# ZijiaLewisLu/CVPR2025-DeCafNet

Measured on AMD Instinct MI355X. Metric: clips/sec (grounding fwd, T=16384 D=1024), higher is better.
Workload: dtype f32; 1 GPU; BASELINE configs[2]: T=16384 D=1024 full multi-scale pyramid + sidekick top-k 30% + expert path, NQ=1 queries/video, 24 independent videos per step: 3 forwards in flight on 3 HIP streams x 8 videos per forward, one replica of this per GPU; T=16384, vid_len=16384, D=1024, E=256, TE=256, levels=8, win=9, heads=4, fusion_layers=2, sn=60, msf=True, norm=True, Lq=32, nq=1, max_batch=8, forwards_in_flight=3

## Files before the change

### cvpr2025-decafnet_amd/_lib.py

```python
import ctypes
import os

_HERE = os.path.dirname(os.path.abspath(__file__))
SO_PATH = os.environ.get('DCF_LIB_PATH') or os.path.join(_HERE, 'libdecafnet_hip.so')
_LIB = None

c_f32p = ctypes.c_void_p
c_u8p = ctypes.c_void_p
c_i32p = ctypes.c_void_p
c_i64p = ctypes.c_void_p
i32, i64, f32, f64 = ctypes.c_int32, ctypes.c_int64, ctypes.c_float, ctypes.c_double
vp = ctypes.c_void_p


class DcfConfig(ctypes.Structure):
    _fields_ = [(n, i32) for n in ('D', 'E', 'TE', 'vid_heads', 'fusion_heads', 'fusion_layers', 'n_embd_convs',
                                   'n_stem', 'n_levels', 'win', 'head_layers', 'sn')] + \
               [('sratio', f32)] + [(n, i32) for n in ('msf', 'norm', 'use_abs_pe', 'max_batch', 'gemm_mode', 'model_kind', 'second_fusion',
                                                      'text_in', 'text_layers', 'text_heads', 'text_abs_pe', 'text_bkgd',
                                                      'scat', 'sfonly', 'text_kind', 'xattn_affine', 'vid_stride', 'pool_only', 'attn_mode')]


class DcfOptimGroup(ctypes.Structure):
    _fields_ = [(n, f32) for n in ('lr', 'weight_decay', 'b1', 'b2', 'one_minus_b1', 'one_minus_b2', 'eps', 'bc1', 'sqrt_bc2')] + [('mode', i32)]
# ... 98 lines not shown
    'dcf_op_decoder': (i32, [vp, ctypes.c_char_p, c_f32p, c_u8p, i32, i32, ctypes.POINTER(vp), ctypes.POINTER(vp), ctypes.POINTER(i32), vp]),
    'dcf_op_tcn': (i32, [vp, ctypes.c_char_p, c_f32p, c_u8p, i32, i32, i32, i32, c_f32p, vp]),
    'dcf_optim_grad_norm': (i32, [vp, c_i32p, i32, i64, f32, c_f32p, c_f32p, vp]),
    'dcf_optim_scale': (i32, [vp, c_i32p, i32, i64, c_f32p, vp]),
    'dcf_optim_adam_step': (i32, [vp, c_i32p, i32, i64, vp, i32, c_f32p, i32, f32, vp]),
}

_DROP = [i32, i32, i32, i32, i64, i32, f32]
TRAIN_SIGNATURES = {
    'dcf_train_ext_version': (i32, []),
    'dcf_op_dropout': (i32, [c_f32p, c_f32p] + _DROP + [vp]),
    'dcf_op_gelu_dropout': (i32, [c_f32p, c_f32p] + _DROP + [vp]),
    'dcf_op_gelu_dropout_bwd': (i32, [c_f32p, c_f32p, c_f32p] + _DROP + [vp]),
    'dcf_op_drop_residual': (i32, [c_f32p, c_u8p, c_f32p, c_u8p, c_f32p, c_f32p] + _DROP + [i32, f32, vp]),
    'dcf_op_drop_residual_bwd': (i32, [c_f32p, c_f32p, c_u8p, c_u8p, c_f32p, c_f32p, c_f32p, c_f32p] + _DROP + [i32, f32, i32, vp]),
}


DIST_SIGNATURES = {
    'dcf_dist_ext_version': (i32, []),
    'dcf_dist_pack_grads': (i32, [vp, c_i32p, i32, i64, f32, vp]),
}


ATTN_SIGNATURES = {
    'dcf_attn_ext_version': (i32, []),
    'dcf_op_global_attn_bwd': (i32, [c_f32p, c_f32p, c_f32p, c_u8p, c_f32p, c_f32p, c_f32p, c_f32p, i32, i32, i32, i32, vp]),
}


FRONT_NO_SKIP = 1
FRONT_SIGNATURES = {
    'dcf_front_ext_version': (i32, []),
    'dcf_op_vidmap_shared': (i32, [c_f32p, c_f32p, c_f32p, c_f32p, c_f32p, c_u8p, c_f32p, c_i32p, c_f32p, i32, i32, i32, i32, i32, vp]),
    'dcf_op_vidmap_shared_bwd': (i32, [c_f32p, c_f32p, c_f32p, c_u8p, c_f32p, c_i32p, c_f32p, c_f32p, c_f32p, i32, i32, i32, i32, i32, i32, vp]),
}


GUARD_APPLY, GUARD_SKIP = 0, 1


class DcfGuardState(ctypes.Structure):
    _fields_ = [('verdict', i32), ('first_bad_row', i32), ('n_bad_rows', i32), ('reserved0', i32), ('applied', i64), ('skipped', i64),
                ('last_skipped_attempt', i64), ('conv_flag', i32), ('reserved1', i32)]


GUARD_SIGNATURES = {
    'dcf_guard_ext_version': (i32, []),
    'dcf_guard_grad_norm': (i32, [vp, c_i32p, i32, i64, f32, c_f32p, c_f32p, vp, vp]),
    'dcf_guard_adam_step': (i32, [vp, c_i32p, i32, i64, vp, i32, c_f32p, vp, i32, f32, vp]),
    'dcf_guard_arm': (i32, [vp, vp]),
    'dcf_guard_disarm': (i32, [vp]),
}


CLOCK_MAX_TABLE = 1 << 22
CLOCK_SIGNATURES = {
    'dcf_clock_ext_version': (i32, []),
    'dcf_clock_adam_step': (i32, [vp, c_i32p, i32, i64, vp, i32, vp, c_i32p, c_i64p, c_f32p, vp, i32, f32, vp]),
}


c_f16p = ctypes.c_void_p
HALF_SIGNATURES = {
    'dcf_half_ext_version': (i32, []),
    'dcf_forward_eval_h': (i32, [vp, c_f16p, c_f16p, c_u8p, i64, i32, ctypes.POINTER(vp), ctypes.POINTER(vp),
                                 ctypes.POINTER(i32), c_f32p, c_f32p, c_f32p, c_u8p, vp]),
    'dcf_forward_eval_videos_h': (i32, [vp, i32, ctypes.POINTER(vp), ctypes.POINTER(vp), ctypes.POINTER(vp), i64, ctypes.POINTER(i32),
                                        ctypes.POINTER(vp), ctypes.POINTER(vp), ctypes.POINTER(i32), ctypes.POINTER(vp),
                                        c_f32p, c_f32p, c_u8p, vp]),
    'dcf_op_linear_cm_split_h': (i32, [c_f16p, c_f32p, c_f32p, c_f32p, i32, i32, i32, i32, i32, vp]),
    'dcf_op_linear_cm_split_ld_h': (i32, [c_f16p, i64, c_f32p, c_f32p, c_f32p, i32, i32, i32, i32, i32, vp]),
    'dcf_op_sidekick_h': (i32, [c_f16p, c_f32p, c_f32p, i32, i32, i32, i32, vp]),
}


FRONT_HALF_SIGNATURES = {
    'dcf_front_half_ext_version': (i32, []),
    'dcf_op_vidmap_shared_h': (i32, [c_f16p, c_f16p, c_f32p, c_f32p, c_f32p, c_u8p, c_f32p, c_i32p, c_f32p, i32, i32, i32, i32, i32, vp]),
    'dcf_op_vidmap_shared_bwd_h': (i32, [c_f16p, c_f16p, c_f32p, c_u8p, c_f32p, c_i32p, c_f32p, c_f32p, c_f32p, i32, i32, i32, i32, i32, i32, vp]),
}


def lib():
    global _LIB
    if _LIB is None:
        import torch
        if not os.path.exists(SO_PATH):
            raise RuntimeError(f'{SO_PATH} is missing: build it with __graft_entry__.build() '
                               f'(there is no CPU fallback for the grounding path)')
        h = ctypes.CDLL(SO_PATH, mode=ctypes.RTLD_GLOBAL)
        for name, (res, args) in list(SIGNATURES.items()) + list(TRAIN_SIGNATURES.items()) + list(DIST_SIGNATURES.items()) + \
                list(ATTN_SIGNATURES.items()) + list(FRONT_SIGNATURES.items()) + list(GUARD_SIGNATURES.items()) + list(CLOCK_SIGNATURES.items()) + \
                list(HALF_SIGNATURES.items()) + list(FRONT_HALF_SIGNATURES.items()):
            fn = getattr(h, name)
            fn.restype = res
            fn.argtypes = args
        _LIB = h
    return _LIB


def check(rc, what=''):
    if rc != 0:
        msg = lib().dcf_last_error().decode(errors='replace')
        raise RuntimeError(f'decafnet_hip {what} failed: {msg}')


def ptr(t):
    return None if t is None else ctypes.c_void_p(t.data_ptr())


def current_stream():
    import torch
    return ctypes.c_void_p(torch.cuda.current_stream().cuda_stream)
```

### cvpr2025-decafnet_amd/csrc/engine.h

```cpp
#pragma once
#include <string>
#include <unordered_map>
#include <vector>

#include "../../include/decafnet_hip.h"
#include "attn.h"
#include "attn_grad.h"
#include "common.h"
#include "dec_chain.h"
#include "dropout.h"
#include "enc_chain.h"
#include "ffn_chain.h"
#include "gemm.h"
#include "head_chain.h"
#include "heads.h"
#include "postproc.h"
#include "rowops.h"
#include "score.h"

namespace dcf {

struct Bound {
  const float* p = nullptr;
  std::vector<int64_t> shape;
  int64_t numel() const {
    int64_t n = 1;
    for (auto s : shape) n *= s;
    return n;
  }
};

struct EncW {
  const float *ln_attn_w, *ln_attn_b, *dw_q, *dw_k, *dw_v, *qn_w, *qn_b, *kn_w, *kn_b, *vn_w, *vn_b;
  const float *wq, *bq, *wk, *bk, *wv, *bv, *wp, *bp, *ls_attn;
  const float *ln_ffn_w, *ln_ffn_b, *fc_w, *fc_b, *pj_w, *pj_b, *ls_ffn;
  const float *fc_wf, *fc_s, *fc_c;
  const unsigned short* qkv_chain[3];
  const float *qkv_s[3], *qkv_c[3];
  const unsigned short* wp_chain;
};
struct DecW {
  const float *ln_q_w, *ln_q_b, *ln_kv_w, *ln_kv_b, *dw, *qn_w, *qn_b;
  const float *wq, *bq, *wk, *bk, *wv, *bv, *wp, *bp;
  const float *wp_il, *bp_il;
  const float *ln_ffn_w, *ln_ffn_b, *fc_w, *fc_b, *pj_w, *pj_b, *ls_ffn;
  const float *fc_wf, *fc_s, *fc_c;
  const unsigned short *wq_chain, *wp_chain;
};
struct TextEncW {
  const float *ln_attn_w, *ln_attn_b, *wq, *bq, *wk, *bk, *wv, *bv, *wp, *bp, *ls_attn;
  const float *ln_ffn_w, *ln_ffn_b, *fc_w, *fc_b, *pj_w, *pj_b, *ls_ffn;
};
struct HeadW {
  std::vector<const float*> conv;
  std::vector<const float*> ln_w, ln_b;
  const float* out_w;
  const float* out_b;
  const unsigned short* chain[2] = {nullptr, nullptr};
  const unsigned short* out_chain = nullptr;
};

static inline int vid_stride_of(const dcf_config& c) { return c.vid_stride > 1 ? c.vid_stride : 1; }

struct Plan {
  int T0 = 0, B = 0, L = 0;
  LevelTable lt{};
  LevelTable* d_lt = nullptr;
};

struct HybridState;

}

struct dcf_model {
  dcf_config cfg{};
  std::unordered_map<std::string, dcf::Bound> bound;
  std::vector<float*> owned;
  std::unordered_map<const float*, const unsigned short*> wsplit;
  std::unordered_map<const float*, int64_t> wsplit_ldw;
  std::unordered_map<const float*, int> wsplit_terms;
  int gemm_terms = 16;
  bool force_x6 = false;
  bool no_ln_carry = false;
  int option_epoch = 0;
  unsigned* status = nullptr;
  bool finalized = false;
  const float* pe = nullptr;
  int64_t pe_T = 0;

  const float *vid_map_w = nullptr, *vid_map_b = nullptr;
  const float *vid_w1 = nullptr, *vid_w2 = nullptr, *vid_w3 = nullptr;
  int64_t vid_ldw = 0;
  std::vector<dcf::DecW> dec;
  const float *fus_out_w = nullptr, *fus_out_b = nullptr;
  const float *embd_fc_w = nullptr, *embd_fc_b = nullptr;
  const float *embd_fc_wf = nullptr, *embd_fc_s = nullptr, *embd_fc_c = nullptr;
  std::vector<const float*> embd_conv, embd_ln_w, embd_ln_b;
  std::vector<dcf::EncW> stem, branch;
  std::vector<const float*> pool_w;
  dcf::HeadW cls1, cls2, reg;
  std::vector<float> reg_scales;
  const float *tcn_in_w = nullptr, *tcn_in_b = nullptr, *tcn_out_w = nullptr, *tcn_out_b = nullptr;
  std::vector<const float*> tcn_wd, tcn_bd, tcn_wp, tcn_bp, tcn_lnw, tcn_lnb;
  std::vector<const unsigned short*> tcn_frag;
  const float *text_embd_w = nullptr, *text_embd_b = nullptr, *text_bkgd = nullptr;
  dcf::TextEncW text_pool{};
  std::vector<dcf::TextEncW> text_enc;
  const float* text_pe = nullptr;
  int64_t text_pe_L = 0;
  char* text_ws = nullptr;
  size_t text_ws_bytes = 0;
  char* half_ws = nullptr;
  size_t half_ws_bytes = 0;

  char* arena = nullptr;
  size_t arena_bytes = 0;
  std::vector<dcf::Plan> plans;
  std::vector<uint64_t> last_key, graph_key;
  hipGraph_t graph = nullptr;
  hipGraphExec_t graph_exec = nullptr;
  bool capturing = false;
  int graph_mode = 0;
  std::vector<uint64_t> nocapture_key;
  int last_launch = 0;
  hipStream_t own = nullptr;
  hipEvent_t ev_in = nullptr, ev_out = nullptr;
  struct {
    float *correl = nullptr, *gate = nullptr, *vidmap = nullptr, *fused = nullptr, *F = nullptr;
    int nq = 0, T0 = 0, B = 0, S = 0;
  } dbg;
  dcf::HybridState* hyb = nullptr;
  int hyb_levels = 0;
  size_t hyb_extra = 0;
  char* hyb_extra_ptr = nullptr;
  float* hyb_feat_out = nullptr;
  float* dbg_vidmap = nullptr;
  float* dbg_fused = nullptr;
  int64_t dbg_cap = 0;
  bool keep_debug = false;
  struct DropState {
    float p[5] = {0.f, 0.f, 0.f, 0.f, 0.f};
    float scale[5] = {1.f, 1.f, 1.f, 1.f, 1.f};
    uint64_t seed = 0;
    bool active = false;
    int b0 = 0;
  } drop_state;
  DropState* drop = nullptr;
};

namespace dcf {

struct Arena {
  char* base;
  size_t off = 0, cap;
  bool dry;
  template <typename T>
  T* take(size_t n) {
    off = (off + 255) & ~(size_t)255;
    T* p = dry ? nullptr : reinterpret_cast<T*>(base + off);
    off += n * sizeof(T);
    return p;
  }
};

struct Buffers {
  float *P1, *P2, *tn, *partial, *correl, *gate;
  uint8_t *mask_all, *nbr_all, *kvmask, *maskv;
  uint8_t* tile_flags;
  uint8_t *mask_pre, *nbr_pre;
  float* col5;
  float *X, *R[7], *H2, *HID, *F, *HA, *HB, *HC, *HD, *logits1, *tcnA, *tcnB, *kvn, *Kt, *Vt;
  unsigned short* kvimg;
  float* kmadd;
  float* stats;
  float* hstats[2];
};

constexpr int DCF_MAX_VIDEOS = 16;
struct VideoSet {
  int nvid = 0;
  const float* vid[DCF_MAX_VIDEOS];
  const float* shallow[DCF_MAX_VIDEOS];
  const uint8_t* mask[DCF_MAX_VIDEOS];
  const float* text_cls[DCF_MAX_VIDEOS];
  int nq[DCF_MAX_VIDEOS];
  float* logits1_out = nullptr;
  bool half = false;
};

struct ForwardCall {
  const float* const* text; const uint8_t* const* text_mask; const int32_t* text_len;
  const float* gate;
  float *logits, *offsets; uint8_t* masks;
};

struct HybridState {
  bool valid = false;
  int k = 0, Tn = 0, Tc = 0, B = 0, Lk = 0;
  Buffers bn{};
  Plan pn{}, pc{}, pch{};
  float *Fc = nullptr, *logits1c = nullptr, *stacked = nullptr;
  uint8_t *maskc = nullptr, *nbrc = nullptr;
};

static inline GemmArgs gemm(const float* A, int64_t lda, const float* W, const float* bias, float* C, int64_t ldc, int M, int N,
                            int K) {
  GemmArgs g{};
  g.A = A; g.lda = lda; g.W = W; g.ldw = 0; g.bias = bias; g.C = C; g.ldc = ldc; g.M = M; g.N = N; g.K = K;
  return g;
}

#define TRY(x) do { if ((x) != 0) return -1; } while (0)
constexpr int STATS_W = 64;
enum { DROP_R_VPROJ = 0, DROP_R_VPATH, DROP_R_FPROJ, DROP_R_FPATH, DROP_R_REFINE };

const char* last_error();
int debug_option(const char* name, int dflt);
int option_epoch();
bool profiling_on();
class Setting {
 public:
  enum Kind { VALUE, PRESENT };
  Setting(const char* opt, const char* env, int dflt, Kind kind = VALUE);
  int get() const;
 private:
  const char* opt_; int base_;
};
void launch_permute3(const float* src, float* dst, int d0, int d1, int d2, int p0, int p1, int p2, hipStream_t st);
void launch_fold_ln(const float* W, const float* bias, const float* g, const float* beta, float* Wf, float* s, float* c, int N, int K,
                    hipStream_t st);
void drop_graph(dcf_model* m, bool keep_last_key = false);
void free_packed(dcf_model* m);
int init_gemm_mode(dcf_model* m, hipStream_t st);
int resolve_encoder(dcf_model* m, const std::string& p, int E, hipStream_t st, EncW& w);
int resolve_decoder(dcf_model* m, const std::string& p, int E, int TE, hipStream_t st, DecW& w);
int resolve_tcn(dcf_model* m, const std::string& pre, int n_in, int n_layers, hipStream_t st);

size_t carve_at(char* base, const dcf_config& c, int T0, int B, int nq, int S, int Lk, int nvid, Buffers& b, size_t extra = 0,
                char** extra_ptr = nullptr);
int get_plan(dcf_model* m, int T0, int B, int L, hipStream_t st, Plan** out);
int make_plan(dcf_model* m, Plan& p, const int* Tl, int n, int B, const float* scales, hipStream_t st);
int run_gemm(dcf_model* m, GemmArgs* g, int count, GemmAMode mode, hipStream_t st);
bool can_fuse_ln(dcf_model* m, const float* W, int M, int N, int K, GemmAMode mode);
bool can_norm_a(dcf_model* m, const float* W1, const float* W2, int M, int C, int* stats_w);
void norm_a(GemmArgs& g, const float* stats, int C, int stats_w, const float* ln_g, const float* ln_b);
EncPreArgs enc_pre_args(const EncW& w, const float* X, int64_t ldx, const uint8_t* mask_in, int B, int T_in, int E);
int run_encoder(dcf_model* m, const EncW& w, Buffers& b, const float* Xin, int64_t ldx, const uint8_t* mask_in,
                const uint8_t* mask_out, int B, int T_in, int stride, float* Xout, int64_t ldo, hipStream_t st);
int run_encoder_drop(dcf_model* m, const EncW& w, Buffers& b, const float* Xin, int64_t ldx, const uint8_t* mask_in,
                     const uint8_t* mask_out, int B, int T_in, int stride, float* Xout, int64_t ldo, uint32_t site0, hipStream_t st);
int run_head(dcf_model* m, const HeadW& h, Buffers& b, const Plan& pl, int Cin, int NO, int mode, int query_major, float* out,
             hipStream_t st, int row0 = 0, int rows = -1);
int run_head_pair(dcf_model* m, const HeadW& h1, const HeadW& h2, Buffers& b, const Plan& pl, int Cin, int NO1, int mode1,
                  float* out1, int NO2, int mode2, float* out2, hipStream_t st);
int run_fusion(dcf_model* m, Buffers& b, float* X, int64_t ldx, int B, int T, const LevelTable* lt, const uint8_t* mask,
               const uint8_t* nbr, const TextMeta* dm, int Lk, float* out, int64_t ld_out, hipStream_t st, bool* carry_out = nullptr);
int run_fusion_drop(dcf_model* m, Buffers& b, float* X, int64_t ldx, int B, int T, const uint8_t* mask, const TextMeta* dm, int Lk,
                    float* out, int64_t ld_out, hipStream_t st);
RefineArgs refine_args(dcf_model* m);

int forward(dcf_model* m, const VideoSet& vs, int T0, int nq, const ForwardCall& fc, hipStream_t st);
void launch_masks_out(const uint8_t* mask_all, uint8_t* out, const LevelTable* lt, const unsigned* status, float* logits, int rows,
                      hipStream_t st);

int launch_half_to_f32(const uint16_t* src, float* dst, int64_t n, hipStream_t st);

void free_hybrid(dcf_model* m);
int hybrid_take(dcf_model* m, const Buffers& b, const Plan& pl, int B, int Lk, hipStream_t st);

}
```

### cvpr2025-decafnet_amd/csrc/engine.hip

```cpp
#include <algorithm>

#include "engine.h"
#include "../../include/decafnet_hip_half.h"

namespace dcf {

__global__ void k_masks_out(const uint8_t* __restrict__ mask_all, uint8_t* __restrict__ out, const LevelTable* lt,
                            const unsigned* __restrict__ status, float* __restrict__ logits) {
  const int r = blockIdx.x * blockDim.x + threadIdx.x;
  const int total = lt->start[lt->n_levels];
  if (r >= total) return;
  int l = 0;
  while (l + 1 < lt->n_levels && r >= lt->start[l + 1]) ++l;
  const int rel = r - lt->start[l];
  const int b = rel / lt->T[l], t = rel - b * lt->T[l];
  const int64_t o = (int64_t)b * lt->S + lt->off[l] + t;
  out[o] = mask_all[r];
  if (status && (status[0] & 3u)) logits[o] = __uint_as_float(0x7fc00000u);
}
void launch_masks_out(const uint8_t* mask_all, uint8_t* out, const LevelTable* lt, const unsigned* status, float* logits, int rows,
                      hipStream_t st) {
  hipLaunchKernelGGL(k_masks_out, dim3((rows + 255) / 256), dim3(256), 0, st, mask_all, out, lt, status, logits);
}

// ... 181 lines not shown
    if (gate_first) {
      if (m->vid_w2) for (int v = 0; v < nvid; ++v) TRY(shallow_half(v));
      TRY(flush());
      TRY(gather_masks());
      GateArgs ga{b.correl, nvid > 1 ? b.maskv : vid_mask, b.gate, sv > 1 ? b.mask_pre : b.mask_all, T0, nq, 0, c.sn, c.msf, (double)c.sratio, vmap0,
                  b.tile_flags, nflags};
      TRY(launch_gate(ga, st));
      auto wit = m->wsplit.find(m->vid_w1);
      const bool one_grid = nvid > 1 && nvid <= GEMM_ZMAX && E % 256 == 0 && T0 % 4 == 0 && wit != m->wsplit.end() && m->wsplit_ldw[m->vid_w1] == m->vid_ldw;
      if (one_grid) {
        GemmArgs base = gemm(vs.vid[0], T0, m->vid_w1, nullptr, b.P1, E, T0, E, D);
        base.ldw = m->vid_ldw; base.a_scale = 1.f; base.Ws = wit->second; base.status = m->status; base.skip_stride = nflags;
        const float* zA[GEMM_ZMAX]; float* zC[GEMM_ZMAX]; const uint8_t* zs[GEMM_ZMAX]; int zq[GEMM_ZMAX];
        for (int v = 0; v < nvid; ++v) { zA[v] = vs.vid[v]; zC[v] = b.P1 + (size_t)v * T0 * E; zs[v] = b.tile_flags + (size_t)q_of[v] * nflags; zq[v] = vs.nq[v]; }
        TRY(launch_gemm_split_z(base, nvid, zA, zC, zs, zq, m->wsplit_terms[m->vid_w1], st, std::min(1.0, std::max(0.0, (double)c.sratio)),
                                half_native ? A_CHANMAJOR_H : A_CHANMAJOR));
      } else {
        for (int v = 0; v < nvid; ++v) TRY(expert_half(v, true));
        TRY(flush());
      }
    } else {
      for (int v = 0; v < nvid; ++v) {
        if (m->vid_w1) TRY(expert_half(v, false));
        if (m->vid_w2) TRY(shallow_half(v));
      }
      TRY(flush());
      TRY(gather_masks());
    }
  }
  if (nvid > 1) vid_mask = b.maskv;

  for (int q0 = 0; q0 < nq; q0 += Bmax) {
    const int B = std::min(Bmax, nq - q0);
    Plan* pl;
    TRY(get_plan(m, Tp, B, L, st, &pl));
    const LevelTable& lt = pl->lt;
    const int rows0 = B * T0, rowsP = B * Tp, rowsAll = B * S;
    uint8_t* mask_in = sv > 1 ? b.mask_pre : b.mask_all;
    if (m->drop) m->drop->b0 = q0;
    unsigned long long vmap = 0;
    for (int i = 0; i < B && i < 16; ++i) vmap |= (unsigned long long)video_of[q0 + i] << (4 * i);

    if (fc.gate) {
      hipLaunchKernelGGL(k_apply_gate, dim3((rows0 + 255) / 256), dim3(256), 0, st, fc.gate + (int64_t)q0 * T0, vid_mask,
                         b.gate, mask_in, T0, rows0, c.msf);
      DCF_HIP(hipGetLastError());
    } else if (!gate_first) {
      GateArgs ga{b.correl, vid_mask, b.gate, mask_in, T0, B, q0, c.sn, c.msf, (double)c.sratio, vmap, nullptr, 0};
      TRY(launch_gate(ga, st));
    }
    int pre_off = 0;
    if (sv > 1) {
      int rows_pre = 0;
      for (int j = 0; j <= npre; ++j) { if (j == npre) pre_off = rows_pre; rows_pre += B * (T0 >> j); }
      TRY(launch_pyramid_masks(b.mask_pre, b.nbr_pre, B, T0, npre + 1, rows_pre, st));
      DCF_HIP(hipMemcpyAsync(b.mask_all, b.mask_pre + pre_off, (size_t)rowsP, hipMemcpyDeviceToDevice, st));
    }
    TRY(launch_pyramid_masks(b.mask_all, b.nbr_all, B, Tp, L, rowsAll, st));
    const uint8_t* mask0 = mask_in;
    const uint8_t* maskP = b.mask_all;

    TRY(launch_vidmap_combine(m->vid_w1 ? b.P1 : nullptr, m->vid_w2 ? b.P2 : nullptr, m->vid_map_b, b.gate, mask0,
                              m->vid_w3, m->vid_w3 ? b.correl + (int64_t)q0 * T0 : nullptr, b.X, T0, rows0, E, vmap, st));
    if (m->keep_debug) DCF_CHECK((int64_t)rows0 * E <= m->dbg_cap, "dcf_debug_copy: armed destination holds %lld floats, the tap needs %lld", (long long)m->dbg_cap, (long long)rows0 * E);
    if (m->keep_debug && m->dbg_vidmap) DCF_HIP(hipMemcpyAsync(m->dbg_vidmap, b.X, (size_t)rows0 * E * 4, hipMemcpyDeviceToDevice, st));

    TextMeta tm{};
    for (int i = 0; i < B; ++i) {
      tm.text[i] = fc.text[q0 + i];
      tm.text_mask[i] = fc.text_mask ? fc.text_mask[q0 + i] : nullptr;
      tm.len[i] = fc.text_len[q0 + i];
    }
    const TextMeta* dm = &tm;

    bool fused_as_stats = false;
    if (c.model_kind != 1) {
      const bool tap = m->keep_debug && m->dbg_fused;
      if (m->drop) TRY(run_fusion_drop(m, b, b.X, E, B, T0, mask0, dm, Lk, b.R[0], E, st));
      else TRY(run_fusion(m, b, b.X, E, B, T0, nullptr, mask0, nullptr, dm, Lk, b.R[0], E, st, tap ? nullptr : &fused_as_stats));
      if (tap) DCF_HIP(hipMemcpyAsync(m->dbg_fused, b.R[0], (size_t)rows0 * E * 4, hipMemcpyDeviceToDevice, st));
    }

    {
      if (c.model_kind != 1 && fused_as_stats) {
        GemmArgs ge = gemm(b.X, E, m->embd_fc_wf, m->embd_fc_c, b.R[3], E, rows0, E, E);
        ge.flags = G_AMASK; ge.rowmask = mask0;
        ge.stats_in = b.stats; ge.ln_s = m->embd_fc_s; ge.stats_slots = E / STATS_W; ge.stats_w = STATS_W;
        TRY(run_gemm(m, &ge, 1, A_ROWS, st));
        std::swap(b.X, b.R[3]);
      } else if (c.model_kind != 1) {
        GemmArgs ge = gemm(b.R[0], E, m->embd_fc_w, m->embd_fc_b, b.X, E, rows0, E, E);
        ge.flags = G_AMASK; ge.rowmask = mask0;
        TRY(run_gemm(m, &ge, 1, A_ROWS, st));
      }
      if (sv > 1) {
        int Tc = T0, off = 0;
        for (int i = 0; i < c.n_embd_convs; ++i) {
          const bool with_pe = c.use_abs_pe && i == c.n_embd_convs - 1;
          if (Tc > Tp) {
            TRY(launch_im2col5s2(b.X, E, b.mask_pre + off, b.col5, B, Tc, E, st));
            GemmArgs g = gemm(b.col5, 5 * E, m->embd_conv[i], nullptr, b.R[0], E, B * (Tc / 2), E, 5 * E);
            TRY(run_gemm(m, &g, 1, A_ROWS, st));
            off += B * Tc;
            Tc /= 2;
          } else {
            GemmArgs g = gemm(b.X, E, m->embd_conv[i], nullptr, b.R[0], E, B * Tc, E, 3 * E);
            g.cin = E; g.nbr = b.nbr_pre + off;
            TRY(run_gemm(m, &g, 1, A_ROWS_TAP3, st));
          }
          LnArgs ln{}; ln.X = b.R[0]; ln.ldx = E; ln.Y = b.X; ln.ldy = E; ln.w = m->embd_ln_w[i]; ln.b = m->embd_ln_b[i];
          ln.rows = B * Tc; ln.C = E; ln.relu = 1;
          if (with_pe) { ln.pe = m->pe; ln.mask = b.mask_pre + off; ln.T = Tc; }
          TRY(launch_ln(ln, st));
        }
        DCF_CHECK(Tc == Tp, "vid_net.arch[0]=%d embedding convolutions cannot divide the sequence by vid_net.stride=%d (video_net.py:53)", c.n_embd_convs, sv);
      }
      int epend = -1, epend_w = 0;
      for (int i = 0; i < c.n_embd_convs && sv == 1; ++i) {
        GemmArgs g = gemm(b.X, E, m->embd_conv[i], nullptr, b.R[0], E, rows0, E, 3 * E);
        g.cin = E; g.nbr = b.nbr_all;
        const bool with_pe = c.use_abs_pe && i == c.n_embd_convs - 1;
        int sw = 0;
        if (epend >= 0) {
          g.A = b.R[0]; g.C = b.R[3];
          norm_a(g, b.hstats[0], E, epend_w, m->embd_ln_w[epend], m->embd_ln_b[epend]);
          epend = -1;
          TRY(run_gemm(m, &g, 1, A_ROWS_TAP3, st));
          LnArgs ln{}; ln.X = b.R[3]; ln.ldx = E; ln.Y = b.X; ln.ldy = E; ln.w = m->embd_ln_w[i]; ln.b = m->embd_ln_b[i];
          ln.rows = rows0; ln.C = E; ln.relu = 1;
          if (with_pe) { ln.pe = m->pe; ln.mask = mask0; ln.T = T0; }
          TRY(launch_ln(ln, st));
        } else if (i + 1 < c.n_embd_convs && i + 2 == c.n_embd_convs && can_norm_a(m, m->embd_conv[i], m->embd_conv[i + 1], rows0, E, &sw)) {
          g.stats_out = b.hstats[0]; g.stats_w = sw;
          TRY(run_gemm(m, &g, 1, A_ROWS_TAP3, st));
          epend = i; epend_w = sw;
        } else
        if (can_fuse_ln(m, m->embd_conv[i], rows0, E, 3 * E, A_ROWS_TAP3)) {
          g.C = nullptr; g.ln_w = m->embd_ln_w[i]; g.ln_b = m->embd_ln_b[i]; g.Y = b.R[3]; g.ldy = E; g.ln_relu = 1;
          if (with_pe) { g.ln_pe = m->pe; g.ln_mask = mask0; g.ln_T = T0; }
          TRY(run_gemm(m, &g, 1, A_ROWS_TAP3, st));
          std::swap(b.X, b.R[3]);
        } else {
          TRY(run_gemm(m, &g, 1, A_ROWS_TAP3, st));
          LnArgs ln{}; ln.X = b.R[0]; ln.ldx = E; ln.Y = b.X; ln.ldy = E; ln.w = m->embd_ln_w[i]; ln.b = m->embd_ln_b[i];
          ln.rows = rows0; ln.C = E; ln.relu = 1;
          if (with_pe) { ln.pe = m->pe; ln.mask = mask0; ln.T = T0; }
          TRY(launch_ln(ln, st));
        }
      }
      if (c.use_abs_pe && c.n_embd_convs == 0) {
        LnArgs ln{}; ln.X = b.X; ln.ldx = E; ln.Y = b.X; ln.ldy = E; ln.rows = rows0; ln.C = E; ln.skip_ln = 1;
        ln.pe = m->pe; ln.mask = mask0; ln.T = T0;
        TRY(launch_ln(ln, st));
      }
      for (size_t i = 0; i < m->stem.size(); ++i) {
        if (m->drop) TRY(run_encoder_drop(m, m->stem[i], b, b.X, E, maskP, maskP, B, Tp, 1, b.R[3], E, drop_site(DROP_G_STEM, (uint32_t)i, 0), st));
        else TRY(run_encoder(m, m->stem[i], b, b.X, E, maskP, maskP, B, Tp, 1, b.R[3], E, st));
        DCF_HIP(hipMemcpyAsync(b.X, b.R[3], (size_t)rowsP * E * 4, hipMemcpyDeviceToDevice, st));
      }
      const int ldf = E + TCN_HID;
      const float* xin = b.X;
      int64_t ldx = E;
      for (int l = 0; l < L; ++l) {
        const int stride = l > 0 ? 2 : 1;
        const uint8_t* mi = b.mask_all + lt.start[l > 0 ? l - 1 : 0];
        const uint8_t* mo = b.mask_all + lt.start[l];
        float* xo = b.F + (int64_t)lt.start[l] * ldf;
        if (c.pool_only) TRY(launch_dwconv3(xin, ldx, mi, m->pool_w[l], xo, ldf, B, l > 0 ? lt.T[l - 1] : Tp, stride, E, st));
        else if (m->drop) TRY(run_encoder_drop(m, m->branch[l], b, xin, ldx, mi, mo, B, l > 0 ? lt.T[l - 1] : Tp, stride, xo, ldf,
                                               drop_site(DROP_G_BRANCH, (uint32_t)l, 0), st));
        else TRY(run_encoder(m, m->branch[l], b, xin, ldx, mi, mo, B, l > 0 ? lt.T[l - 1] : Tp, stride, xo, ldf, st));
        xin = xo; ldx = ldf;
      }
    }

    if (m->hyb_levels > 0) {
      TRY(hybrid_take(m, b, *pl, B, Lk, st));
      continue;
    }

    if (c.model_kind == 1 || c.second_fusion)
      TRY(run_fusion(m, b, b.F, E + TCN_HID, B, Tp, &lt, b.mask_all, b.nbr_all, dm, Lk, b.F, E + TCN_HID, st));

    if (c.model_kind != 0) {
      TRY(run_head_pair(m, m->cls1, m->reg, b, *pl, E, 1, 0, fc.logits + (int64_t)q0 * S, 2, 1, fc.offsets + (int64_t)q0 * S * 2, st));
    } else {
    TRY(run_head(m, m->cls1, b, *pl, E, 1, 0, 0, b.logits1, st));
    if (vs.logits1_out) {
      hipLaunchKernelGGL(k_points_out, dim3((rowsAll + 255) / 256), dim3(256), 0, st, (const float*)b.logits1,
                         vs.logits1_out + (int64_t)q0 * S, (const LevelTable*)pl->d_lt);
      DCF_HIP(hipGetLastError());
    }
    {
      RefineArgs ra = refine_args(m);
      ra.logits1 = b.logits1; ra.lt = pl->d_lt; ra.mask_all = b.mask_all;
      ra.bufA = b.tcnA; ra.bufB = b.tcnB; ra.F = b.F; ra.ldf = E + TCN_HID; ra.E = E;
      ra.B = B; ra.T0 = Tp; ra.n_levels = L; ra.n_layers = L;
      if (m->drop) {
        ra.drop_seed = m->drop->seed; ra.drop_p = m->drop->p[DROP_R_REFINE]; ra.drop_scale = m->drop->scale[DROP_R_REFINE]; ra.drop_b0 = q0;
      }
      TRY(launch_refine(ra, lt, st));
// ... 291 lines not shown
```

### cvpr2025-decafnet_amd/csrc/engine_blocks.hip

```cpp
#include <algorithm>

#include "engine.h"

namespace dcf {

static void carve(Arena& a, const dcf_config& c, int T0, int B, int nq, int S, int Lk, int nvid, Buffers& b) {
  const size_t rows0 = (size_t)B * T0, rowsAll = (size_t)B * S;
  const size_t rowsF = std::max(rows0, (c.model_kind == 1 || c.second_fusion) ? rowsAll : (size_t)0);
  const bool strided = vid_stride_of(c) > 1;
  const int E = c.E, EH = c.E + TCN_HID;
  b.P1 = a.take<float>((size_t)nvid * T0 * E);
  b.P2 = a.take<float>((size_t)nvid * T0 * E);
  b.maskv = a.take<uint8_t>(nvid > 1 ? (size_t)nvid * T0 : 0);
  b.tn = a.take<float>((size_t)nq * c.D);
  b.partial = a.take<float>((size_t)SCORE_SLICES * (nq + nvid) * T0);
  b.correl = a.take<float>((size_t)nq * T0);
  b.gate = a.take<float>(rows0);
  b.tile_flags = a.take<uint8_t>((size_t)B * ((T0 + 63) / 64));
  b.mask_all = a.take<uint8_t>(rowsAll);
  b.nbr_all = a.take<uint8_t>(rowsAll);
  b.mask_pre = a.take<uint8_t>(strided ? 2 * rows0 : 0);
  b.nbr_pre = a.take<uint8_t>(strided ? 2 * rows0 : 0);
  b.col5 = a.take<float>(strided ? rows0 / 2 * 5 * E : 0);
  b.kvmask = a.take<uint8_t>((size_t)B * Lk);
// ... 463 lines not shown
  }
  if (!m->fus_out_w) return 0;
  LnArgs ln{}; ln.X = X; ln.ldx = ldx; ln.Y = out; ln.ldy = ld_out; ln.w = m->fus_out_w; ln.b = m->fus_out_b; ln.rows = rows; ln.C = E;
  TRY(launch_ln(ln, st));
  return 0;
}

static DropSite drop_at(const dcf_model* m, int rate, uint32_t site) {
  DropSite d;
  d.site = site; d.p = m->drop->p[rate]; d.scale = m->drop->scale[rate];
  return d;
}

int run_encoder_drop(dcf_model* m, const EncW& w, Buffers& b, const float* Xin, int64_t ldx, const uint8_t* mask_in,
                     const uint8_t* mask_out, int B, int T_in, int stride, float* Xout, int64_t ldo, uint32_t site0,
                     hipStream_t st) {
  const dcf_config& c = m->cfg;
  const int E = c.E, To = T_in / stride, rows = B * To;
  const auto& d = *m->drop;
  TRY(enc_unfused_qkv(m, w, b, Xin, ldx, mask_in, B, T_in, stride, st));
  TRY(enc_unfused_attention(m, b, mask_out, B, To, st));
  GemmArgs gp = gemm(b.R[0], E, w.wp, w.bp, b.R[4], E, rows, E, E);
  TRY(run_gemm(m, &gp, 1, A_ROWS, st));
  DropResArgs ra{};
  ra.out = b.R[1]; ra.ldo = E;
  if (stride == 2) { ra.R = b.R[3]; ra.ldr = E; } else { ra.R = Xin; ra.ldr = ldx; }
  ra.H = b.R[4]; ra.ldh = E; ra.rowmask = mask_out; ra.res_mask = 1; ra.out_mask = 0; ra.ls = w.ls_attn;
  ra.rows = rows; ra.C = E; ra.T = To; ra.b0 = d.b0; ra.seed = d.seed;
  ra.drop = drop_at(m, DROP_R_VPROJ, site0 | DROP_PROJ); ra.path = drop_at(m, DROP_R_VPATH, site0 | DROP_PATH_ATTN);
  TRY(launch_drop_residual(ra, st));
  LnArgs ln{}; ln.X = b.R[1]; ln.ldx = E; ln.Y = b.R[2]; ln.ldy = E; ln.w = w.ln_ffn_w; ln.b = w.ln_ffn_b; ln.rows = rows; ln.C = E;
  TRY(launch_ln(ln, st));
  GemmArgs gf = gemm(b.R[2], E, w.fc_w, w.fc_b, b.HID, 4 * E, rows, 4 * E, E);
  gf.flags = G_GELU;
  TRY(run_gemm(m, &gf, 1, A_ROWS, st));
  TRY(launch_dropout(b.HID, 4 * E, rows, 4 * E, To, d.b0, d.seed, drop_at(m, DROP_R_VPROJ, site0 | DROP_FFN_HID), st));
  GemmArgs go = gemm(b.HID, 4 * E, w.pj_w, w.pj_b, b.R[4], E, rows, E, 4 * E);
  TRY(run_gemm(m, &go, 1, A_ROWS, st));
  ra.out = Xout; ra.ldo = ldo; ra.R = b.R[1]; ra.ldr = E; ra.res_mask = 0; ra.out_mask = 1; ra.ls = w.ls_ffn;
  ra.drop = drop_at(m, DROP_R_VPROJ, site0 | DROP_FFN_OUT); ra.path = drop_at(m, DROP_R_VPATH, site0 | DROP_PATH_FFN);
  return launch_drop_residual(ra, st);
}

int run_fusion_drop(dcf_model* m, Buffers& b, float* X, int64_t ldx, int B, int T, const uint8_t* mask, const TextMeta* dm,
                    int Lk, float* out, int64_t ld_out, hipStream_t st) {
  const dcf_config& c = m->cfg;
  const int E = c.E, rows = B * T;
  const auto& d = *m->drop;
  for (size_t li = 0; li < m->dec.size(); ++li) {
    const DecW& w = m->dec[li];
    const uint32_t site0 = drop_site(DROP_G_FUSION, (uint32_t)li, 0);
    TextLnArgs tl{*dm, b.kvn, b.kvmask, w.ln_kv_w, w.ln_kv_b, Lk, c.TE};
    TRY(launch_text_ln(tl, B, st));
    GemmArgs gkv[2] = {gemm(b.kvn, c.TE, w.wk, w.bk, b.Kt, E, B * Lk, E, c.TE), gemm(b.kvn, c.TE, w.wv, w.bv, b.Vt, E, B * Lk, E, c.TE)};
    TRY(run_gemm(m, gkv, 2, A_ROWS, st));
    DecPreArgs dp{X, ldx, mask, w.ln_q_w, w.ln_q_b, w.dw, w.qn_w, w.qn_b, b.R[0], b.R[1], B, T, E};
    dp.nbr = nullptr;
    dp.affine = c.xattn_affine;
    TRY(launch_dec_pre(dp, st));
    GemmArgs gq = gemm(b.R[0], E, w.wq, w.bq, b.R[2], E, rows, E, E);
    TRY(run_gemm(m, &gq, 1, A_ROWS, st));
    XAttnArgs xa{b.R[2], b.Kt, b.Vt, b.kvmask, b.R[0], B, T, Lk, E, c.fusion_heads, m->status, c.attn_mode == 1};
    TRY(launch_xattn(xa, st));
    GemmArgs gh = gemm(b.R[0], E, w.wp, w.bp, b.H2, 2 * E, rows, 2 * E, E);
    TRY(run_gemm(m, &gh, 1, A_ROWS, st));
    TRY(launch_dropout(b.H2, 2 * E, rows, 2 * E, T, d.b0, d.seed, drop_at(m, DROP_R_FPROJ, site0 | DROP_PROJ), st));
    TRY(launch_dec_mid(b.R[1], b.H2, w.ln_ffn_w, w.ln_ffn_b, b.R[2], b.R[0], rows, E, st));
    GemmArgs gf = gemm(b.R[0], E, w.fc_w, w.fc_b, b.HID, 4 * E, rows, 4 * E, E);
    gf.flags = G_GELU;
    TRY(run_gemm(m, &gf, 1, A_ROWS, st));
    TRY(launch_dropout(b.HID, 4 * E, rows, 4 * E, T, d.b0, d.seed, drop_at(m, DROP_R_FPROJ, site0 | DROP_FFN_HID), st));
    GemmArgs go = gemm(b.HID, 4 * E, w.pj_w, w.pj_b, b.R[1], E, rows, E, 4 * E);
    TRY(run_gemm(m, &go, 1, A_ROWS, st));
    DropResArgs ra{};
    ra.out = X; ra.ldo = ldx; ra.R = b.R[2]; ra.ldr = E; ra.H = b.R[1]; ra.ldh = E; ra.rowmask = mask; ra.res_mask = 0; ra.out_mask = 1;
    ra.ls = w.ls_ffn; ra.rows = rows; ra.C = E; ra.T = T; ra.b0 = d.b0; ra.seed = d.seed;
    ra.drop = drop_at(m, DROP_R_FPROJ, site0 | DROP_FFN_OUT); ra.path = drop_at(m, DROP_R_FPATH, site0 | DROP_PATH_FFN);
    TRY(launch_drop_residual(ra, st));
  }
  LnArgs ln{}; ln.X = X; ln.ldx = ldx; ln.Y = out; ln.ldy = ld_out; ln.w = m->fus_out_w; ln.b = m->fus_out_b; ln.rows = rows; ln.C = E;
  return launch_ln(ln, st);
}

RefineArgs refine_args(dcf_model* m) {
  static const Setting stack("tcn_stack", "DCF_TCN_STACK", -1);
  RefineArgs ra{};
  ra.w_in = m->tcn_in_w; ra.b_in = m->tcn_in_b;
  ra.host_w_dil = m->tcn_wd.data(); ra.host_b_dil = m->tcn_bd.data(); ra.host_w_pw = m->tcn_wp.data();
  ra.host_b_pw = m->tcn_bp.data(); ra.host_ln_w = m->tcn_lnw.data(); ra.host_ln_b = m->tcn_lnb.data();
  ra.w_out = m->tcn_out_w; ra.b_out = m->tcn_out_b;
  ra.host_frag = (!m->tcn_frag.empty() && debug_option("tcn_frag", 1) != 0) ? m->tcn_frag.data() : nullptr;
  ra.stack_layers = stack.get();
  ra.f16 = m->gemm_terms == GEMM_F16X3; ra.status = m->status;
  return ra;
}

}
```

### cvpr2025-decafnet_amd/csrc/engine_model.hip

```cpp
#include <cstdarg>
#include <cstdio>
#include <cstdlib>
#include <algorithm>
#include <cstring>
#include <atomic>
#include <mutex>

#include "engine.h"

namespace dcf {

static thread_local std::string g_err;
void set_error(const char* fmt, ...) {
  char buf[1024];
  va_list ap;
  va_start(ap, fmt);
  vsnprintf(buf, sizeof(buf), fmt, ap);
  va_end(ap);
  g_err = buf;
}
const char* last_error() { return g_err.c_str(); }

static std::unordered_map<std::string, int>& debug_options() {
  static std::unordered_map<std::string, int> o;
  return o;
}
static std::mutex& debug_options_mutex() {
  static std::mutex mu;
  return mu;
}
static std::atomic<int> g_option_epoch{0};
int option_epoch() { return g_option_epoch.load(); }
int debug_option(const char* name, int dflt) {
  std::lock_guard<std::mutex> lock(debug_options_mutex());
  auto& o = debug_options();
  auto it = o.find(name);
  return it == o.end() ? dflt : it->second;
}
Setting::Setting(const char* opt, const char* env, int dflt, Kind kind) : opt_(opt), base_(dflt) {
  const char* v = env ? getenv(env) : nullptr;
  if (v) base_ = kind == PRESENT ? 1 : atoi(v);
}
int Setting::get() const { return opt_ ? debug_option(opt_, base_) : base_; }

struct ProfRec { std::string name; hipEvent_t a, b; double flops, bytes; };
static bool g_prof_on = false;
static std::vector<ProfRec> g_recs;
bool profiling_on() { return g_prof_on; }

ProfScope::ProfScope(const char* name, hipStream_t s, double flops, double bytes) : idx(-1), st(s) {
  if (!g_prof_on) return;
  ProfRec r{name, nullptr, nullptr, flops, bytes};
  if (hipEventCreate(&r.a) != hipSuccess || hipEventCreate(&r.b) != hipSuccess) return;
  (void)hipEventRecord(r.a, st);
  g_recs.push_back(r);
  idx = (int)g_recs.size() - 1;
}
ProfScope::~ProfScope() {
  if (idx >= 0) (void)hipEventRecord(g_recs[idx].b, st);
}

__global__ void k_permute3(const float* __restrict__ src, float* __restrict__ dst, int d0, int d1, int d2, int p0, int p1,
                           int p2) {
  const int n = d0 * d1 * d2;
  const int i = blockIdx.x * blockDim.x + threadIdx.x;
  if (i >= n) return;
  int idx[3];
  idx[0] = i / (d1 * d2);
  idx[1] = (i / d2) % d1;
  idx[2] = i % d2;
  const int dims[3] = {d0, d1, d2};
  const int perm[3] = {p0, p1, p2};
  const int o = (idx[perm[0]] * dims[perm[1]] + idx[perm[1]]) * dims[perm[2]] + idx[perm[2]];
  dst[o] = src[i];
}
void launch_permute3(const float* src, float* dst, int d0, int d1, int d2, int p0, int p1, int p2, hipStream_t st) {
  const size_t n = (size_t)d0 * d1 * d2;
  hipLaunchKernelGGL(k_permute3, dim3((unsigned)((n + 255) / 256)), dim3(256), 0, st, src, dst, d0, d1, d2, p0, p1, p2);
}

__global__ __launch_bounds__(64) void k_fold_ln(const float* __restrict__ W, const float* __restrict__ bias, const float* __restrict__ g,
                                                const float* __restrict__ beta, float* __restrict__ Wf, float* __restrict__ s,
                                                float* __restrict__ c, int K) {
  const int n = blockIdx.x, lane = threadIdx.x;
  float a1 = 0.f, a2 = 0.f;
  for (int k = lane; k < K; k += 64) {
    const float w = W[(int64_t)n * K + k];
    const float wf = w * g[k];
    Wf[(int64_t)n * K + k] = wf;
    a1 += wf;
    a2 += beta[k] * w;
  }
  a1 = wave_sum(a1);
  a2 = wave_sum(a2);
  if (lane == 0) { s[n] = a1; c[n] = (bias ? bias[n] : 0.f) + a2; }
}
void launch_fold_ln(const float* W, const float* bias, const float* g, const float* beta, float* Wf, float* s, float* c, int N, int K,
                    hipStream_t st) {
  hipLaunchKernelGGL(k_fold_ln, dim3(N), dim3(64), 0, st, W, bias, g, beta, Wf, s, c, K);
}

void drop_graph(dcf_model* m, bool keep_last_key) {
  if (m->graph_exec) (void)hipGraphExecDestroy(m->graph_exec);
  if (m->graph) (void)hipGraphDestroy(m->graph);
  m->graph_exec = nullptr;
  m->graph = nullptr;
  m->graph_key.clear();
  if (!keep_last_key) m->last_key.clear();
}

void free_packed(dcf_model* m) {
  for (float* p : m->owned) (void)hipFree(p);
  m->owned.clear();
  m->wsplit.clear();
  m->wsplit_ldw.clear();
  m->wsplit_terms.clear();
}

static int free_model(dcf_model* m) {
  drop_graph(m);
  if (m->status) (void)hipFree(m->status);
  m->status = nullptr;
  free_packed(m);
  for (auto& pl : m->plans) if (pl.d_lt) (void)hipFree(pl.d_lt);
  m->plans.clear();
  free_hybrid(m);
  if (m->arena) (void)hipFree(m->arena);
  if (m->text_ws) (void)hipFree(m->text_ws);
  if (m->half_ws) (void)hipFree(m->half_ws);
  if (m->ev_in) (void)hipEventDestroy(m->ev_in);
  if (m->ev_out) (void)hipEventDestroy(m->ev_out);
  if (m->own) (void)hipStreamDestroy(m->own);
  return 0;
}

static int get(dcf_model* m, const std::string& name, std::initializer_list<int64_t> shape, const float** out) {
  auto it = m->bound.find(name);
  DCF_CHECK(it != m->bound.end(), "parameter '%s' is not bound", name.c_str());
  const Bound& b = it->second;
  int64_t want = 1;
  for (auto s : shape) want *= s;
  DCF_CHECK(b.numel() == want, "parameter '%s' has %lld elements, expected %lld", name.c_str(), (long long)b.numel(),
            (long long)want);
  *out = b.p;
  return 0;
}

static int pack3(dcf_model* m, const float* src, int d0, int d1, int d2, int p0, int p1, int p2, hipStream_t st,
                 const float** out) {
  float* dst = nullptr;
  const size_t n = (size_t)d0 * d1 * d2;
  DCF_HIP(hipMalloc(&dst, n * sizeof(float)));
  m->owned.push_back(dst);
  launch_permute3(src, dst, d0, d1, d2, p0, p1, p2, st);
  DCF_HIP(hipGetLastError());
  *out = dst;
  return 0;
}

static int split_weight(dcf_model* m, const float* W, int N, int K, hipStream_t st, int64_t ldw = 0, int terms = 0) {
  if (m->gemm_terms == 0 || m->wsplit.count(W)) return 0;
  if (!terms) terms = m->gemm_terms;
  unsigned short* planes = nullptr;
  DCF_HIP(hipMalloc(&planes, (size_t)3 * N * K * sizeof(unsigned short)));
  m->owned.push_back(reinterpret_cast<float*>(planes));
  if (launch_split_planes(W, planes, N, K, ldw ? ldw : K, st, terms, m->status ? m->status + 1 : nullptr)) return -1;
  m->wsplit[W] = planes;
  m->wsplit_ldw[W] = ldw ? ldw : K;
  m->wsplit_terms[W] = terms;
  return 0;
}
#define SPLIT(W, N, K) do { if (split_weight(m, (W), (N), (K), st)) return -1; } while (0)

static int fold_ln(dcf_model* m, const float* W, const float* bias, const float* g, const float* beta, int N, int K, hipStream_t st,
                   const float** wf, const float** s_out, const float** c_out) {
  float* buf = nullptr;
  DCF_HIP(hipMalloc(&buf, ((size_t)N * K + 2 * (size_t)N) * sizeof(float)));
  m->owned.push_back(buf);
  float* sv = buf + (size_t)N * K;
  launch_fold_ln(W, bias, g, beta, buf, sv, sv + N, N, K, st);
  DCF_HIP(hipGetLastError());
  *wf = buf; *s_out = sv; *c_out = sv + N;
// ... 208 lines not shown
      const std::string p = "text_net.attn_pool.attn";
      GET(p + ".query.weight", SH(TE, TE), w.wq); GET(p + ".query.bias", SH(TE), w.bq);
      GET(p + ".key.weight", SH(TE, TE), w.wk); GET(p + ".key.bias", SH(TE), w.bk);
      GET(p + ".value.weight", SH(TE, TE), w.wv); GET(p + ".value.bias", SH(TE), w.bv);
      GET(p + ".proj.weight", SH(TE, TE), w.wp); GET(p + ".proj.bias", SH(TE), w.bp);
      SPLIT(w.wq, TE, TE); SPLIT(w.wk, TE, TE); SPLIT(w.wv, TE, TE); SPLIT(w.wp, TE, TE);
    }
  } else
  if (c.text_layers > 0 || c.text_in > 0) {
    DCF_CHECK(c.text_in > 0 && c.text_layers >= 0 && c.text_heads >= 1 && TE % c.text_heads == 0,
              "text_net: in_dim=%d layers=%d heads=%d do not fit TE=%d", c.text_in, c.text_layers, c.text_heads, TE);
    GET("text_net.embd_fc.conv.weight", SH(TE, c.text_in), m->text_embd_w); GET("text_net.embd_fc.conv.bias", SH(TE), m->text_embd_b);
    if (c.text_bkgd) GET("text_net.bkgd_token", SH(TE), m->text_bkgd);
    for (int i = 0; i < c.text_layers; ++i) {
      const std::string p = "text_net.transformer." + std::to_string(i);
      TextEncW w{};
      GET(p + ".ln_attn.weight", SH(TE), w.ln_attn_w); GET(p + ".ln_attn.bias", SH(TE), w.ln_attn_b);
      GET(p + ".attn.attn.query.weight", SH(TE, TE), w.wq); GET(p + ".attn.attn.query.bias", SH(TE), w.bq);
      GET(p + ".attn.attn.key.weight", SH(TE, TE), w.wk); GET(p + ".attn.attn.key.bias", SH(TE), w.bk);
      GET(p + ".attn.attn.value.weight", SH(TE, TE), w.wv); GET(p + ".attn.attn.value.bias", SH(TE), w.bv);
      GET(p + ".attn.attn.proj.weight", SH(TE, TE), w.wp); GET(p + ".attn.attn.proj.bias", SH(TE), w.bp);
      GET(p + ".drop_path_attn.scale", SH(TE), w.ls_attn);
      GET(p + ".ln_ffn.weight", SH(TE), w.ln_ffn_w); GET(p + ".ln_ffn.bias", SH(TE), w.ln_ffn_b);
      GET(p + ".ffn.fc.weight", SH(4 * TE, TE), w.fc_w); GET(p + ".ffn.fc.bias", SH(4 * TE), w.fc_b);
      GET(p + ".ffn.proj.weight", SH(TE, 4 * TE), w.pj_w); GET(p + ".ffn.proj.bias", SH(TE), w.pj_b);
      GET(p + ".drop_path_ffn.scale", SH(TE), w.ls_ffn);
      SPLIT(w.wq, TE, TE); SPLIT(w.wk, TE, TE); SPLIT(w.wv, TE, TE); SPLIT(w.wp, TE, TE);
      SPLIT(w.fc_w, 4 * TE, TE); SPLIT(w.pj_w, TE, 4 * TE);
      m->text_enc.push_back(w);
    }
  }

  if (c.model_kind == 1) {
    GET("vid_net.embd_fc.conv.weight", SH(E, Din), m->vid_map_w); GET("vid_net.embd_fc.conv.bias", SH(E), m->vid_map_b);
  } else {
    GET("vid_map.conv.weight", SH(E, Din), m->vid_map_w); GET("vid_map.conv.bias", SH(E), m->vid_map_b);
  }
  m->vid_w1 = (c.msf && sfonly) ? nullptr : m->vid_map_w;
  m->vid_w2 = c.msf ? (sfonly ? m->vid_map_w : m->vid_map_w + D) : nullptr;
  m->vid_w3 = nullptr;
  m->vid_ldw = Din;
  if (c.scat) {
    float* blk[3] = {nullptr, nullptr, nullptr};
    const float* src[3] = {m->vid_w1, m->vid_w2, m->vid_map_w + (Din - 1)};
    const int wid[3] = {D, D, 1};
    for (int i = 0; i < 3; ++i) {
      if (!src[i]) continue;
      DCF_HIP(hipMalloc(&blk[i], (size_t)E * wid[i] * sizeof(float)));
      m->owned.push_back(blk[i]);
      DCF_HIP(hipMemcpy2DAsync(blk[i], (size_t)wid[i] * 4, src[i], (size_t)Din * 4, (size_t)wid[i] * 4, E, hipMemcpyDeviceToDevice, st));
    }
    m->vid_w1 = blk[0]; m->vid_w2 = blk[1]; m->vid_w3 = blk[2];
    m->vid_ldw = D;
  }
  if (D % 32 == 0 && E % 32 == 0) {
    if (m->vid_w1 && split_weight(m, m->vid_w1, E, D, st, m->vid_ldw)) return -1;
    if (m->vid_w2 && split_weight(m, m->vid_w2, E, D, st, m->vid_ldw)) return -1;
  }
  for (int i = 0; i < c.fusion_layers; ++i) {
    DecW w{};
    if (resolve_decoder(m, "fusion.layers." + std::to_string(i), E, TE, st, w)) return -1;
    m->dec.push_back(w);
  }
  GET("fusion.ln_out.weight", SH(E), m->fus_out_w); GET("fusion.ln_out.bias", SH(E), m->fus_out_b);
  if (c.model_kind != 1) {
    GET("vid_net.embd_fc.conv.weight", SH(E, E), m->embd_fc_w); GET("vid_net.embd_fc.conv.bias", SH(E), m->embd_fc_b);
    SPLIT(m->embd_fc_w, E, E);
    m->embd_fc_wf = m->embd_fc_s = m->embd_fc_c = nullptr;
    if (m->gemm_terms != 0 && E % 64 == 0 && c.fusion_layers > 0 &&
        fold_ln(m, m->embd_fc_w, m->embd_fc_b, m->fus_out_w, m->fus_out_b, E, E, st, &m->embd_fc_wf, &m->embd_fc_s, &m->embd_fc_c)) return -1;
  }
  for (int i = 0, sv = vid_stride_of(c); i < c.n_embd_convs; ++i, sv = std::max(sv / 2, 1)) {
    const std::string s = std::to_string(i);
    const int taps = sv > 1 ? 5 : 3;
    GET("vid_net.embd_convs." + s + ".conv.weight", SH(E, E, taps), t);
    const float* pk;
    if (pack3(m, t, E, E, taps, 0, 2, 1, st, &pk)) return -1;
    SPLIT(pk, E, taps * E);
    m->embd_conv.push_back(pk);
    const float *lw, *lb;
    GET("vid_net.embd_norms." + s + ".weight", SH(E), lw); GET("vid_net.embd_norms." + s + ".bias", SH(E), lb);
    m->embd_ln_w.push_back(lw); m->embd_ln_b.push_back(lb);
  }
  for (int i = 0; i < c.n_stem; ++i) {
    EncW w{};
    if (resolve_encoder(m, "vid_net.stem." + std::to_string(i), E, st, w)) return -1;
    m->stem.push_back(w);
  }
  m->pool_w.clear();
  for (int i = 0; i < L; ++i) {
    if (c.pool_only) {
      const float* pk;
      GET("vid_net.branch." + std::to_string(i) + ".conv.weight", SH(E, 3), t);
      if (pack3(m, t, 1, E, 3, 0, 2, 1, st, &pk)) return -1;
      m->pool_w.push_back(pk);
      continue;
    }
    EncW w{};
    if (resolve_encoder(m, "vid_net.branch." + std::to_string(i), E, st, w)) return -1;
    m->branch.push_back(w);
  }
  if (resolve_head(m, "cls_head", "cls_head", E, 1, c.head_layers, st, m->cls1)) return -1;
  const int EH = c.model_kind == 0 ? E + TCN_HID : E;
  if (c.model_kind == 0 && resolve_head(m, "cls_head2", "cls_head", EH, 1, c.head_layers, st, m->cls2)) return -1;
  if (resolve_head(m, "reg_head", "reg_head", EH, 2, c.head_layers, st, m->reg)) return -1;
  m->reg_scales.assign(L, 1.f);
  for (int l = 0; l < L; ++l) {
    GET("reg_head.scales." + std::to_string(l) + ".scale", SH(1), t);
    DCF_HIP(hipMemcpyAsync(&m->reg_scales[l], t, sizeof(float), hipMemcpyDeviceToHost, st));
  }
  if (c.model_kind == 0 && resolve_tcn(m, "refine", L, L, st)) return -1;
  DCF_HIP(hipStreamSynchronize(st));
  for (auto& pl : m->plans) if (pl.d_lt) (void)hipFree(pl.d_lt);
  m->plans.clear();
  free_hybrid(m);
  drop_graph(m);
  if (m->gemm_terms == GEMM_F16X3) {
    unsigned flags[2] = {0u, 0u};
    DCF_HIP(hipMemcpyAsync(flags, m->status, sizeof(flags), hipMemcpyDeviceToHost, st));
    DCF_HIP(hipStreamSynchronize(st));
    if (flags[1]) {
      m->force_x6 = true;
      return finalize(m, st);
    }
  }
  m->finalized = true;
  return 0;
}

}

extern "C" {

int dcf_model_create(const dcf_config* cfg, dcf_model** out) {
  DCF_CHECK(cfg && out, "dcf_model_create: null argument");
  DCF_CHECK(cfg->E > 0 && cfg->E % 32 == 0 && cfg->E <= 992, "E=%d must be a positive multiple of 32 (<= 992)", cfg->E);
  DCF_CHECK(cfg->attn_mode == 0 || cfg->attn_mode == 1, "attn_mode=%d: 0 (f16x3) or 1 (one fp16 product)", cfg->attn_mode);
  DCF_CHECK(cfg->D > 0 && cfg->D % 32 == 0, "D=%d must be a positive multiple of 32", cfg->D);
  DCF_CHECK(cfg->TE > 0 && cfg->TE % 32 == 0, "TE=%d must be a positive multiple of 32", cfg->TE);
  DCF_CHECK(cfg->n_levels >= 1 && cfg->n_levels <= dcf::DCF_MAX_LEVELS, "n_levels=%d out of range", cfg->n_levels);
  DCF_CHECK(cfg->win == 0 || (cfg->win > 0 && (cfg->win & 1)), "mha_win_size=%d must be odd, or 0 for global self-attention over the clips", cfg->win);
  DCF_CHECK(cfg->fusion_layers >= 0 && cfg->head_layers >= 0 && cfg->n_embd_convs >= 0 && cfg->n_stem >= 0, "negative layer count");
  DCF_CHECK(cfg->sn >= 1, "sn must be >= 1");
  DCF_CHECK(cfg->model_kind >= 0 && cfg->model_kind <= 2, "model_kind must be 0 (iterative early fusion), 1 (late fusion) or 2 (early fusion)");
  {
    const int sv = cfg->vid_stride > 1 ? cfg->vid_stride : 1;
    int lg = 0;
    while ((1 << lg) < sv) ++lg;
    DCF_CHECK((sv & (sv - 1)) == 0 && cfg->n_embd_convs >= lg, "vid_net.stride=%d must be a power of two with arch[0]=%d >= log2(stride) (video_net.py:52-53)",
              sv, cfg->n_embd_convs);
  }
  int ndev = 0;
  DCF_HIP(hipGetDeviceCount(&ndev));
  DCF_CHECK(ndev > 0, "no HIP device");
  dcf_model* m = new dcf_model();
  m->cfg = *cfg;
  *out = m;
  return 0;
}

void dcf_model_destroy(dcf_model* m) {
  if (!m) return;
  dcf::free_model(m);
  delete m;
}

int dcf_model_bind(dcf_model* m, const char* name, const float* data, const int64_t* shape, int32_t ndim) {
  DCF_CHECK(m && name && data, "dcf_model_bind: null argument");
  dcf::Bound b;
  b.p = data;
  for (int i = 0; i < ndim; ++i) b.shape.push_back(shape[i]);
  m->bound[name] = b;
  m->finalized = false;
  return 0;
}

int dcf_model_set_pe(dcf_model* m, const float* pe_tokens, int64_t T) {
  DCF_CHECK(m, "dcf_model_set_pe: null model");
  m->pe = pe_tokens;
  m->pe_T = T;
  return 0;
}

int dcf_model_set_text_pe(dcf_model* m, const float* pe_tokens, int64_t L) {
  DCF_CHECK(m, "dcf_model_set_text_pe: null model");
  m->text_pe = pe_tokens;
  m->text_pe_L = L;
  return 0;
}

int dcf_model_finalize(dcf_model* m, void* stream) {
  DCF_CHECK(m, "dcf_model_finalize: null model");
  return dcf::finalize(m, (hipStream_t)stream);
}

int dcf_numerics_status(dcf_model* m, int32_t reset, void* stream) {
  DCF_CHECK(m, "dcf_numerics_status: null model");
  int out = m->gemm_terms == dcf::GEMM_BF16X6 ? 4 : (m->gemm_terms == 0 ? 8 : 0);
  if (m->force_x6) out |= 2;
  if (m->status) {
    unsigned flag = 0u;
    hipStream_t st = (hipStream_t)stream;
    DCF_HIP(hipMemcpyAsync(&flag, m->status, sizeof(flag), hipMemcpyDeviceToHost, st));
    if (reset) DCF_HIP(hipMemsetAsync(m->status, 0, sizeof(unsigned), st));
    DCF_HIP(hipStreamSynchronize(st));
    if (flag & ~2u) out |= 1;
    if (flag & 2u) out |= 16;
  }
  return out;
}

int dcf_model_set_ln_carry(dcf_model* m, int32_t on) {
  DCF_CHECK(m, "dcf_model_set_ln_carry: null model");
  const bool off = on == 0;
  if (off != m->no_ln_carry) dcf::drop_graph(m);
  m->no_ln_carry = off;
  return 0;
}

int dcf_numerics_status_async(dcf_model* m, int32_t* host_dst, void* stream) {
  DCF_CHECK(m && host_dst, "dcf_numerics_status_async: null argument");
  if (!m->status) { *host_dst = 0; return 0; }
  DCF_HIP(hipMemcpyAsync(host_dst, m->status, sizeof(unsigned), hipMemcpyDeviceToHost, (hipStream_t)stream));
  return 0;
}

int dcf_model_set_dropout(dcf_model* m, float vid_proj_p, float vid_path_p, float fus_proj_p, float fus_path_p, float refine_p,
                          int64_t seed) {
  DCF_CHECK(m, "dcf_model_set_dropout: null model");
  const float p[5] = {vid_proj_p, vid_path_p, fus_proj_p, fus_path_p, refine_p};
  for (int i = 0; i < 5; ++i) DCF_CHECK(p[i] >= 0.f && p[i] < 1.f, "dcf_model_set_dropout: rate %d = %g outside [0, 1)", i, (double)p[i]);
  auto& d = m->drop_state;
  d.active = false;
  for (int i = 0; i < 5; ++i) {
    d.p[i] = p[i];
    d.scale[i] = 1.0f / (1.0f - p[i]);
    d.active = d.active || p[i] > 0.f;
  }
  d.seed = (uint64_t)seed;
  return 0;
}

int dcf_debug_set_option(const char* name, int32_t value) {
  DCF_CHECK(name && *name, "dcf_debug_set_option: empty name");
  static const char* known[] = {"dec_chain_min_rows", "enc_chain_min_rows", "enc_attn_min_rows", "fuse_scores", "tcn_frag", "gate_skip", "tcn_stack", "half_native"};
  bool ok = false;
  for (const char* k : known) ok = ok || strcmp(k, name) == 0;
  DCF_CHECK(ok, "dcf_debug_set_option: unknown option '%s'", name);
  {
    std::lock_guard<std::mutex> lock(dcf::debug_options_mutex());
    if (value < 0) dcf::debug_options().erase(name);
    else dcf::debug_options()[name] = value;
  }
  dcf::g_option_epoch.fetch_add(1);
  return 0;
}

int dcf_model_set_graph_mode(dcf_model* m, int32_t mode) {
  DCF_CHECK(m && mode >= 0 && mode <= 2, "dcf_model_set_graph_mode: mode must be 0 (auto), 1 (always) or 2 (never)");
  if (mode != m->graph_mode) dcf::drop_graph(m);
  m->graph_mode = mode;
  return 0;
}

int dcf_debug_copy(dcf_model* m, int32_t what, float* dst, int64_t max_floats, void* stream) {
  DCF_CHECK(m && dst, "dcf_debug_copy: null argument");
  hipStream_t st = (hipStream_t)stream;
  const float* src = nullptr;
  int64_t n = 0;
  const int E = m->cfg.E;
  switch (what) {
    case 0: src = m->dbg.correl; n = (int64_t)m->dbg.nq * m->dbg.T0; break;
    case 1: src = m->dbg.gate; n = (int64_t)m->dbg.B * m->dbg.T0; break;
    case 4: src = m->dbg.F; n = (int64_t)m->dbg.B * m->dbg.S * (E + dcf::TCN_HID); break;
    case 2: case 3: {
      m->keep_debug = true;
      m->dbg_cap = max_floats;
      if (what == 2) m->dbg_vidmap = dst; else m->dbg_fused = dst;
      return 0;
    }
    default: DCF_CHECK(false, "dcf_debug_copy: unknown selector %d", what);
  }
  DCF_CHECK(src, "dcf_debug_copy: no forward has run yet");
  DCF_CHECK(n <= max_floats, "dcf_debug_copy: destination too small (%lld > %lld)", (long long)n, (long long)max_floats);
  DCF_HIP(hipMemcpyAsync(dst, src, n * sizeof(float), hipMemcpyDeviceToDevice, st));
  return 0;
}

int dcf_profile_enable(int32_t on) {
  for (auto& r : dcf::g_recs) { (void)hipEventDestroy(r.a); (void)hipEventDestroy(r.b); }
  dcf::g_recs.clear();
  dcf::g_prof_on = on != 0;
  return 0;
}

int64_t dcf_profile_report(char* buf, int64_t cap) {
  struct Agg { long count = 0; double ms = 0, flops = 0, bytes = 0; };
  std::vector<std::pair<std::string, Agg>> aggs;
  for (auto& r : dcf::g_recs) {
    if (hipEventSynchronize(r.b) != hipSuccess) continue;
    float ms = 0.f;
    if (hipEventElapsedTime(&ms, r.a, r.b) != hipSuccess) continue;
    Agg* a = nullptr;
    for (auto& kv : aggs) if (kv.first == r.name) a = &kv.second;
    if (!a) { aggs.emplace_back(r.name, Agg()); a = &aggs.back().second; }
    a->count++; a->ms += ms; a->flops += r.flops; a->bytes += r.bytes;
  }
  std::string out = "{";
  for (size_t i = 0; i < aggs.size(); ++i) {
    char line[512];
    snprintf(line, sizeof(line), "%s\"%s\": {\"count\": %ld, \"ms\": %.6f, \"flops\": %.6e, \"bytes\": %.6e}", i ? ", " : "",
             aggs[i].first.c_str(), aggs[i].second.count, aggs[i].second.ms, aggs[i].second.flops, aggs[i].second.bytes);
    out += line;
  }
  out += "}";
  if (buf && cap > 0) {
    size_t n = std::min((size_t)cap - 1, out.size());
    memcpy(buf, out.data(), n);
    buf[n] = 0;
  }
  return (int64_t)out.size() + 1;
}

}
```

### cvpr2025-decafnet_amd/csrc/gemm_bf16s.hip

```cpp
#include <cstdio>
#include <type_traits>
#include <cstdlib>

#include "gemm_common.h"


namespace dcf {

typedef __bf16 bf16x8 __attribute__((ext_vector_type(8)));
typedef __bf16 bf16x2 __attribute__((ext_vector_type(2)));
typedef float f32x2 __attribute__((ext_vector_type(2)));
typedef unsigned int u32x4 __attribute__((ext_vector_type(4)));

typedef _Float16 f16x8 __attribute__((ext_vector_type(8)));
typedef _Float16 f16x2 __attribute__((ext_vector_type(2)));
typedef _Float16 f16x4 __attribute__((ext_vector_type(4)));

constexpr int SBK = 32;
constexpr int ROWB = 80;

constexpr int T_F16 = 16;
constexpr float F16_SA = 16.f, F16_SW = 256.f, F16_UNSCALE = 1.f / 4096.f;

__device__ __forceinline__ void split2(float x0, float x1, unsigned& hi, unsigned& mid, unsigned& lo) {
// ... 639 lines not shown
    if constexpr (BN % 64 == 0 && !(WM == 2 && TM == 2)) {
      if (nterms == 6) {
        if constexpr (DEEP) hipLaunchKernelGGL((gemm_bf16s_kernel<WM, WN, TM, TN, A_ROWS, 6, false, 2, true>), grid, dim3(WM * WN * 64), lds, stream, b);
        else hipLaunchKernelGGL((gemm_bf16s_kernel<WM, WN, TM, TN, A_ROWS, 6, false, 2, true>), grid, dim3(WM * WN * 64), lds, stream, b);
      } else {
        if constexpr (DEEP) hipLaunchKernelGGL((gemm_bf16s_kernel<WM, WN, TM, TN, A_ROWS, T_F16, false, 3, true>), grid, dim3(WM * WN * 64), lds, stream, b);
        else hipLaunchKernelGGL((gemm_bf16s_kernel<WM, WN, TM, TN, A_ROWS, T_F16, false, 2, true>), grid, dim3(WM * WN * 64), lds, stream, b);
      }
    } else {
      DCF_CHECK(false, "launch_gemm_split: no row-statistics kernel for %dx%d tiles", BM, BN);
    }
  } else
  if (p.ln_w) {
    if constexpr (WM == 1 && TM == 2 && TN >= 2) {
      DCF_CHECK(mode != A_CHANMAJOR && mode != A_CHANMAJOR_H && count == 1, "launch_gemm_split: fused LayerNorm: unsupported mode");
      if (mode == A_ROWS) { if (nterms == 6) LSN(A_ROWS, 6); else LSN(A_ROWS, T_F16); }
      else { if (nterms == 6) LSN(A_ROWS_TAP3, 6); else LSN(A_ROWS_TAP3, T_F16); }
    } else {
      DCF_CHECK(false, "launch_gemm_split: fused LayerNorm is not built for this tile");
    }
  } else
  if (mode == A_ROWS) { if (nterms == 6) LS(A_ROWS, 6); else LS(A_ROWS, T_F16); }
  else if (mode == A_ROWS_TAP3) { if (nterms == 6) LS(A_ROWS_TAP3, 6); else LS(A_ROWS_TAP3, T_F16); }
  else {
    if constexpr (WM == 1 && WN == 4 && TM == 2) {
      bool want_score = false;
      int score_q = 0;
      for (int i = 0; i < count && i < 3; ++i) {
        if (!b.g[i].score_out) continue;
        want_score = true;
        DCF_CHECK(b.g[i].score_tn && b.g[i].score_nq >= 1 && b.g[i].score_nq <= GEMM_SCORE_MAXQ && b.g[i].M % 4 == 0 &&
                  (reinterpret_cast<uintptr_t>(b.g[i].score_out) & 15) == 0, "launch_gemm_split: bad score arguments (1 .. %d queries)", GEMM_SCORE_MAXQ);
        score_q = b.g[i].score_nq > score_q ? b.g[i].score_nq : score_q;
      }
      if (want_score) {
        const size_t lds_sc = lds + (size_t)score_q * p.K * sizeof(float);
        DCF_CHECK(lds_sc <= 65536, "launch_gemm_split: %d text vectors of %d channels beside the tile need %zu bytes of LDS (> 64 KiB)", score_q, p.K, lds_sc);
        constexpr int NST_ = DEEP ? 3 : 2;
        if (mode == A_CHANMAJOR_H) {
          if (nterms == 6) hipLaunchKernelGGL((gemm_bf16s_kernel<WM, WN, TM, TN, A_CHANMAJOR_H, 6, false, 2, false, false, true>), grid, dim3(WM * WN * 64), lds_sc, stream, b);
          else hipLaunchKernelGGL((gemm_bf16s_kernel<WM, WN, TM, TN, A_CHANMAJOR_H, T_F16, false, NST_, false, false, true>), grid, dim3(WM * WN * 64), lds_sc, stream, b);
        } else
        if (nterms == 6) hipLaunchKernelGGL((gemm_bf16s_kernel<WM, WN, TM, TN, A_CHANMAJOR, 6, false, 2, false, false, true>), grid, dim3(WM * WN * 64), lds_sc, stream, b);
        else hipLaunchKernelGGL((gemm_bf16s_kernel<WM, WN, TM, TN, A_CHANMAJOR, T_F16, false, NST_, false, false, true>), grid, dim3(WM * WN * 64), lds_sc, stream, b);
      } else if (mode == A_CHANMAJOR_H) {
        if (nterms == 6) LS(A_CHANMAJOR_H, 6); else LS(A_CHANMAJOR_H, T_F16);
      } else {
        if (nterms == 6) LS(A_CHANMAJOR, 6); else LS(A_CHANMAJOR, T_F16);
      }
    }
    else DCF_CHECK(false, "launch_gemm_split: channel-major A needs a 64-row tile");
  }
#undef LS
#undef LSN
#undef LSK
  DCF_HIP(hipGetLastError());
  return 0;
}

static int launch_kslice(const GemmBatch& b, int count, int nterms, hipStream_t stream) {
  const GemmArgs& p = b.g[0];
  constexpr long small_max = 128;
  const long tiles64 = (long)((p.M + 63) / 64) * (p.N / 64) * count;
  const bool small = tiles64 <= small_max;
  dim3 grid(small ? tile_grid<32, 64>(p) : tile_grid<64, 64>(p), 1, count);
  char name[96];
  static const bool shapes = getenv("DCF_PROF_SHAPES") != nullptr;
  const char* fam = nterms == 6 ? "gemm_bf16x6" : "gemm_f16x3";
  if (shapes) snprintf(name, sizeof(name), "%s<%dx64,kslice>[%dx%dx%dx%d]", fam, small ? 32 : 64, count, p.M, p.N, p.K);
  else snprintf(name, sizeof(name), "%s<64x64,kslice>", fam);
  const double mnk = (double)count * p.M * (double)p.N * p.K;
  ProfScope prof(name, stream, 2.0 * mnk, 4.0 * count * ((double)p.M * p.K + 1.5 * (double)p.N * p.K + (double)p.M * p.N * ((p.flags & G_RES) ? 2 : 1)));
  if (small) {
    if (nterms == 6) hipLaunchKernelGGL((gemm_bf16s_kslice_kernel<6, 1>), grid, dim3(256), 0, stream, b);
    else hipLaunchKernelGGL((gemm_bf16s_kslice_kernel<T_F16, 1>), grid, dim3(256), 0, stream, b);
  } else {
    if (nterms == 6) hipLaunchKernelGGL((gemm_bf16s_kslice_kernel<6, 2>), grid, dim3(256), 0, stream, b);
    else hipLaunchKernelGGL((gemm_bf16s_kslice_kernel<T_F16, 2>), grid, dim3(256), 0, stream, b);
  }
  DCF_HIP(hipGetLastError());
  return 0;
}

bool gemm_can_fuse_adaln(int M, int N, int K) {
  if (N % 256 != 0 || K % SBK != 0) return false;
  const long tiles64 = (long)((M + 63) / 64) * (N / 64);
  if (K >= 4 * SBK && tiles64 <= 512) return false;
  return M >= 65536 || (long)((M + 63) / 64) * (N / 256) >= 448;
}

bool gemm_can_carry_stats(int M, int N, int K, int count, int nterms) {
  if (nterms == 0 || N % 64 != 0 || K % SBK != 0 || M <= 0) return false;
  const long tiles64 = (long)((M + 63) / 64) * (N / 64) * count;
  constexpr long kslice_max = 512;
  if (K >= 4 * SBK && tiles64 <= ((K >= 16 * SBK && nterms != T_F16) ? kslice_max : kslice_max / 2)) return false;
  return true;
}

bool gemm_can_norm_a(int M, int N, int K, int nterms, int* stats_w) {
  if (nterms == 0 || K % SBK != 0 || M <= 0) return false;
  if (N % 256 == 0 && M >= 65536) { if (stats_w) *stats_w = 64; return true; }
  (void)nterms;
  return false;
}

bool gemm_can_fuse_ln(int M, int N, int K, GemmAMode mode) {
  constexpr long min_tiles = 448;
  return mode != A_CHANMAJOR && mode != A_CHANMAJOR_H && N == 256 && K % SBK == 0 && (M + 63) / 64 >= min_tiles;
}

int launch_gemm_split(const GemmArgs* g, int count, GemmAMode mode, int nterms, hipStream_t stream) {
  DCF_CHECK(count >= 1 && count <= 3, "launch_gemm_split: count %d out of range", count);
  DCF_CHECK(nterms == T_F16 || nterms == 6, "launch_gemm_split: nterms must be 16 (f16x3) or 6 (bf16x6)");
  GemmBatch b{};
  for (int i = 0; i < 3; ++i) b.g[i] = g[i < count ? i : 0];
  if (mode == A_ROWS_TAP3)
    for (int i = 0; i < 3; ++i) b.g[i].flags |= G_TAPSLAB;
  const GemmArgs& p = g[0];
  for (int i = 0; i < count; ++i) {
    DCF_CHECK(g[i].M == p.M && g[i].N == p.N && g[i].K == p.K, "launch_gemm_split: grouped shapes differ");
    DCF_CHECK(g[i].A && g[i].Ws && (g[i].C || (g[i].ln_w && g[i].Y)), "launch_gemm_split: null operand");
    DCF_CHECK(g[i].lda % 4 == 0, "launch_gemm_split: lda %% 4 != 0");
    if (mode == A_CHANMAJOR || mode == A_CHANMAJOR_H) DCF_CHECK(g[i].M % 4 == 0 && !(g[i].flags & G_AMASK), "launch_gemm_split: channel-major A needs M %% 4 == 0, no row mask");
    if (mode == A_CHANMAJOR_H) {
      DCF_CHECK((reinterpret_cast<uintptr_t>(g[i].A) & 7) == 0, "launch_gemm_split: half channel-major A needs an 8-byte aligned base (and lda %% 4 == 0, M %% 4 == 0)");
      DCF_CHECK(!g[i].ln_w && !g[i].stats_out && !g[i].stats_in, "launch_gemm_split: half channel-major A carries neither a fused LayerNorm nor row statistics");
    }
    if (mode == A_ROWS_TAP3) DCF_CHECK(g[i].nbr && g[i].cin % 32 == 0 && g[i].K == 3 * g[i].cin, "launch_gemm_split: bad tap3 args");
    if (g[i].flags & (G_AMASK | G_RES_MASK | G_OUT_MASK)) DCF_CHECK(g[i].rowmask, "launch_gemm_split: rowmask missing");
    if (g[i].flags & G_RES) DCF_CHECK(g[i].R, "launch_gemm_split: residual missing");
    if (g[i].stats_out || g[i].stats_in) {
      int sw_ = 0;
      DCF_CHECK((mode == A_ROWS && gemm_can_carry_stats(g[i].M, g[i].N, g[i].K, count, nterms)) ||
                (mode == A_ROWS_TAP3 && !g[i].stats_in && gemm_can_norm_a(g[i].M, g[i].N, g[i].K, nterms, &sw_) && sw_ == g[i].stats_w),
                "launch_gemm_split: row statistics: %dx%dx%d (x%d) runs on a kernel without them", g[i].M, g[i].N, g[i].K, count);
      DCF_CHECK(g[i].ldc % 4 == 0 && (reinterpret_cast<uintptr_t>(g[i].C) & 15) == 0 && (!g[i].bias || (reinterpret_cast<uintptr_t>(g[i].bias) & 15) == 0) &&
                (!(g[i].flags & G_RES) || (g[i].ldr % 4 == 0 && (reinterpret_cast<uintptr_t>(g[i].R) & 15) == 0 && (!g[i].ls || (reinterpret_cast<uintptr_t>(g[i].ls) & 15) == 0))) &&
                (!g[i].stats_in || (g[i].ln_s && (reinterpret_cast<uintptr_t>(g[i].ln_s) & 15) == 0 && g[i].stats_slots >= 1)) && g[i].stats_w > 0 && !g[i].ln_w,
                "launch_gemm_split: row statistics need 16-byte aligned C / R / bias / ls / ln_s, stats_w > 0 and no fused LayerNorm");
    }
    if (g[i].flags & G_ADALN)
      DCF_CHECK(g[i].flags == G_ADALN && mode == A_ROWS && g[i].R && !g[i].ln_w && g[i].ldc % 4 == 0 && g[i].ldr % 4 == 0 &&
                (reinterpret_cast<uintptr_t>(g[i].C) & 15) == 0 && (reinterpret_cast<uintptr_t>(g[i].R) & 15) == 0 &&
                (!g[i].bias || (reinterpret_cast<uintptr_t>(g[i].bias) & 15) == 0) && gemm_can_fuse_adaln(g[i].M, g[i].N, g[i].K),
                "launch_gemm_split: G_ADALN needs A_ROWS, a residual, 16-byte aligned C / R, no other epilogue flag and a tile-kernel grid");
  }
  if (p.M <= 0) return 0;
  DCF_CHECK(p.K > 0 && p.K % SBK == 0 && p.N > 0 && p.N % 32 == 0, "launch_gemm_split: bad N=%d / K=%d", p.N, p.K);
  const int N = p.N;
  auto wgs = [&](int bm, int bn) { return (long)((p.M + bm - 1) / bm) * (N / bn) * count; };
  constexpr long WANT = 448;
  static const char* forced = getenv("DCF_GEMM_CFG");
  if (forced) {
    int bm = 0, bn = 0;
    if (sscanf(forced, "%dx%d", &bm, &bn) == 2 && bn > 0 && N % bn == 0) {
      if (bm == 64 && bn == 256) return launch_cfg_s<1, 4, 2, 2>(b, count, mode, nterms, stream);
      if (bm == 64 && bn == 128) return launch_cfg_s<1, 4, 2, 1>(b, count, mode, nterms, stream);
      if (bm == 64 && bn == 64) return launch_cfg_s<2, 2, 1, 1>(b, count, mode, nterms, stream);
      if (bm == 128 && bn == 128) return launch_cfg_s<2, 2, 2, 2>(b, count, mode, nterms, stream);
      if (bm == 128 && bn == 256) return launch_cfg_s<1, 4, 4, 2>(b, count, mode, nterms, stream);
    }
  }
  if (p.ln_w) {
    DCF_CHECK(count == 1 && p.Y && p.ln_b && gemm_can_fuse_ln(p.M, N, p.K, mode), "launch_gemm_split: LayerNorm cannot be fused for %dx%dx%d", p.M, N, p.K);
    if (p.ln_pe) DCF_CHECK(p.ln_mask && p.ln_T >= 64, "launch_gemm_split: fused position encoding needs a mask and T >= 64");
    return launch_cfg_s<1, 4, 2, 2>(b, count, mode, nterms, stream);
  }
  constexpr long kslice_max = 512;
  if (mode == A_ROWS && N % 64 == 0 && p.K >= 4 * SBK && wgs(64, 64) <= ((p.K >= 16 * SBK && nterms != T_F16) ? kslice_max : kslice_max / 2))
    return launch_kslice(b, count, nterms, stream);
  if (mode == A_CHANMAJOR || mode == A_CHANMAJOR_H) {
    DCF_CHECK(N % 128 == 0, "launch_gemm_split: channel-major A needs N %% 128 == 0");
    if (N % 256 == 0 && wgs(64, 256) >= WANT) return launch_cfg_s<1, 4, 2, 2>(b, count, mode, nterms, stream);
    return launch_cfg_s<1, 4, 2, 1>(b, count, mode, nterms, stream);
  }
  if (N % 256 == 0 && p.M >= 65536 && mode != A_CHANMAJOR && mode != A_CHANMAJOR_H) return launch_cfg_s<1, 4, 4, 2>(b, count, mode, nterms, stream);
  if (N % 256 == 0 && wgs(64, 256) >= WANT) return launch_cfg_s<1, 4, 2, 2>(b, count, mode, nterms, stream);
  if (N % 96 == 0 && N % 64 != 0) {
    if (nterms == T_F16) return launch_cfg_s<1, 3, 4, 1>(b, count, mode, nterms, stream);
    return launch_cfg_s<4, 1, 1, 3>(b, count, mode, nterms, stream);
  }
  if (N % 160 == 0 && N % 64 != 0) return launch_cfg_s<4, 1, 1, 5>(b, count, mode, nterms, stream);
  if (N % 128 == 0 && wgs(64, 128) >= WANT) return launch_cfg_s<1, 4, 2, 1>(b, count, mode, nterms, stream);
  if (N % 64 == 0) return launch_cfg_s<2, 2, 1, 1>(b, count, mode, nterms, stream);
  return launch_cfg_s<4, 1, 1, 1>(b, count, mode, nterms, stream);
}

int launch_gemm_split_z(const GemmArgs& base, int nz, const float* const* A, float* const* C, const uint8_t* const* skip, const int* skip_nq,
                        int nterms, hipStream_t stream, double work_fraction, GemmAMode mode) {
  DCF_CHECK(mode == A_CHANMAJOR || mode == A_CHANMAJOR_H, "launch_gemm_split_z: a channel-major A mode only");
  DCF_CHECK(nz >= 1 && nz <= GEMM_ZMAX, "launch_gemm_split_z: %d operand sets (1 .. %d)", nz, GEMM_ZMAX);
  DCF_CHECK(nterms == T_F16 || nterms == 6, "launch_gemm_split_z: nterms must be 16 (f16x3) or 6 (bf16x6)");
  DCF_CHECK(base.Ws && base.M > 0 && base.M % 4 == 0 && base.N % 256 == 0 && base.K > 0 && base.K % SBK == 0 && base.lda % 4 == 0 && !base.flags &&
                !base.score_out && !base.ln_w && !base.stats_out && !base.stats_in,
            "launch_gemm_split_z: a plain channel-major GEMM with N %% 256 == 0 only");
  GemmBatch b{};
  for (int i = 0; i < 3; ++i) b.g[i] = base;
  b.zcount = nz;
  for (int z = 0; z < nz; ++z) {
    DCF_CHECK(A[z] && C[z], "launch_gemm_split_z: null operand");
    if (mode == A_CHANMAJOR_H) DCF_CHECK((reinterpret_cast<uintptr_t>(A[z]) & 7) == 0, "launch_gemm_split_z: half channel-major A needs an 8-byte aligned base");
    b.zA[z] = A[z]; b.zC[z] = C[z]; b.zskip[z] = skip ? skip[z] : nullptr; b.zskip_nq[z] = skip && skip[z] ? skip_nq[z] : 0;
  }
  b.g[0].A = A[0]; b.g[0].C = C[0];
  return launch_cfg_s<1, 4, 2, 2>(b, nz, mode, nterms, stream, work_fraction);
}

}
```

### cvpr2025-decafnet_amd/csrc/head_chain.hip

```cpp
#include "head_chain.h"

#include <type_traits>

#include "common.h"

namespace dcf {

namespace {

typedef _Float16 f16x8 __attribute__((ext_vector_type(8)));
typedef _Float16 f16x2 __attribute__((ext_vector_type(2)));
typedef float f32x2 __attribute__((ext_vector_type(2)));
typedef unsigned u32x4 __attribute__((ext_vector_type(4)));

constexpr float SA = 16.f, SW = 256.f, UNSCALE = 1.f / 4096.f;
constexpr int HALO = 3, WGROWS = 128, VALID = WGROWS - 2 * HALO;

template <int C>
struct Geo {
  static constexpr int KS = C / 16;
  static constexpr int KH = KS / 2;
  static constexpr int NT = C / 32;
  static constexpr int PIECES = 3 * KH * 2;
  static constexpr int STAGE = PIECES * 1024;
  static constexpr int SPL = 2 * NT;
  static constexpr int NPW = (PIECES + 3) / 4;
  static_assert(C % 32 == 0 && KS % 2 == 0, "C must be a multiple of 32");
};

__device__ __forceinline__ void split2_f16(float x0, float x1, float s, unsigned& hi, unsigned& lo) {
  const f16x2 h = __builtin_convertvector(f32x2{x0 * s, x1 * s}, f16x2);
  hi = __builtin_bit_cast(unsigned, h);
  const float r0 = __builtin_fmaf(x0, s, -(float)h[0]), r1 = __builtin_fmaf(x1, s, -(float)h[1]);
  lo = __builtin_bit_cast(unsigned, __builtin_convertvector(f32x2{r0, r1}, f16x2));
}

__device__ __forceinline__ void glds16(const void* sbase, unsigned voff, unsigned lds_dst) {
#ifdef DCF_GLDS_KEEP_M0
  unsigned keep;
  asm volatile("s_mov_b32 %0, m0\n\ts_mov_b32 m0, %3\n\ts_nop 0\n\tglobal_load_lds_dwordx4 %1, %2\n\ts_mov_b32 m0, %0"
               : "=&s"(keep)
               : "v"(voff), "s"(sbase), "s"(lds_dst)
               : "memory");
#else
  asm volatile("s_mov_b32 m0, %2\n\ts_nop 0\n\tglobal_load_lds_dwordx4 %0, %1" : : "v"(voff), "s"(sbase), "s"(lds_dst) : "memory");
#endif
}

#ifdef DCF_HC_STAMP
__device__ unsigned long long dcf_hc_stamps[8];
__device__ __forceinline__ unsigned long long hc_stamp() {
  unsigned long long t;
  __builtin_amdgcn_sched_barrier(0);
  asm volatile("s_memtime %0\n\ts_waitcnt lgkmcnt(0)" : "=s"(t) : : "memory");
  __builtin_amdgcn_sched_barrier(0);
  return t;
}
#define STAMP(i) do { const unsigned long long t_ = hc_stamp(); acc_[i] += t_ - last_; last_ = t_; } while (0)
#else
#define STAMP(i) do { } while (0)
#endif

__device__ __forceinline__ f32x16 mma(f16x8 a, f16x8 b, f32x16 c) { return __builtin_amdgcn_mfma_f32_32x32x16_f16(a, b, c, 0, 0, 0); }

__device__ __forceinline__ float from_prev(float v) { return __int_as_float(__builtin_amdgcn_update_dpp(0, __float_as_int(v), 0x138, 0xf, 0xf, true)); }
__device__ __forceinline__ float from_next(float v) { return __int_as_float(__builtin_amdgcn_update_dpp(0, __float_as_int(v), 0x130, 0xf, 0xf, true)); }

__device__ __forceinline__ int find_level_hc(const LevelTable* lt, int r) {
  int l = 0;
  while (l + 1 < lt->n_levels && r >= lt->start[l + 1]) ++l;
  return l;
}

}

template <int C>
__global__ void k_split_chain3(const float* __restrict__ Wp, unsigned short* __restrict__ img, unsigned* __restrict__ overflow) {
  using G = Geo<C>;
  const int i = blockIdx.x * blockDim.x + threadIdx.x;
  if (i >= C * 3 * (C / 2)) return;
  const int n = i / (3 * (C / 2)), rem = i - n * (3 * (C / 2)), tap = rem / (C / 2), k = (rem - tap * (C / 2)) * 2;
  const float w0 = Wp[((size_t)n * 3 + tap) * C + k], w1 = Wp[((size_t)n * 3 + tap) * C + k + 1];
  unsigned hi, lo;
  split2_f16(w0, w1, SW, hi, lo);
  if (!(__builtin_fabsf(w0) * SW <= 65504.f) || !(__builtin_fabsf(w1) * SW <= 65504.f)) {
    if (overflow) atomicOr(overflow, 1u);
  }
  const int ot = n >> 5, rr = n & 31, kk = k >> 4, hf = kk / G::KH, kq = kk - hf * G::KH, kr = k & 15;
  const int a = kr >> 3, h = (kr >> 2) & 1, ii = kr & 3, j = 4 * a + ii;
  const size_t piece = (size_t)(ot * 2 + hf) * G::PIECES + (size_t)(tap * G::KH + kq) * 2;
  const size_t o = (piece * 64 + h * 32 + rr) * 8 + j;
  *reinterpret_cast<unsigned*>(img + o) = hi;
  *reinterpret_cast<unsigned*>(img + o + 64 * 8) = lo;
}

template <int C>
__global__ void k_split_chain_out(const float* __restrict__ Wout, int NO, unsigned short* __restrict__ img, unsigned* __restrict__ overflow) {
  const int i = blockIdx.x * blockDim.x + threadIdx.x;
  if (i >= 6 * (C / 2)) return;
  const int e = i / (C / 2), k = (i - e * (C / 2)) * 2, tap = e >> 1, o = e & 1;
  if (o >= NO) return;
  const float w0 = Wout[((size_t)o * 3 + tap) * C + k], w1 = Wout[((size_t)o * 3 + tap) * C + k + 1];
  unsigned hi, lo;
  split2_f16(w0, w1, SW, hi, lo);
  if (!(__builtin_fabsf(w0) * SW <= 65504.f) || !(__builtin_fabsf(w1) * SW <= 65504.f)) {
    if (overflow) atomicOr(overflow, 1u);
  }
  const int rr = 8 * (e >> 2) + (e & 3), kk = k >> 4, kr = k & 15;
  const int a = kr >> 3, h = (kr >> 2) & 1, ii = kr & 3, j = 4 * a + ii;
  const size_t o_ = ((size_t)(2 * kk) * 64 + h * 32 + rr) * 8 + j;
  *reinterpret_cast<unsigned*>(img + o_) = hi;
  *reinterpret_cast<unsigned*>(img + o_ + 64 * 8) = lo;
}

struct HeadChainBatch { HeadChainArgs a[2]; };
template <int C>
__global__ __launch_bounds__(256, 1) void k_head_chain(HeadChainBatch batch) {
  constexpr int NO = 2;
  const HeadChainArgs& p = batch.a[blockIdx.y];
  using G = Geo<C>;
  constexpr int KS = G::KS, KH = G::KH, NT = G::NT, STAGE = G::STAGE, PIECES = G::PIECES, NPW = G::NPW;
  extern __shared__ __attribute__((aligned(16))) unsigned char lds[];
  float* lds_ln = reinterpret_cast<float*>(lds + 2 * STAGE);
#ifdef DCF_HC_VECTOR_OUT
  float* lds_wo = lds_ln + 4 * C;
  float* lds_x = lds_wo + NO * 3 * C;
#else
  float* lds_x = lds_ln + 4 * C;
#endif
  const int tid = threadIdx.x, lane = tid & 63, r = lane & 31, h = lane >> 5;
  const int w = __builtin_amdgcn_readfirstlane(tid >> 6);
  const unsigned lane16 = (unsigned)lane * 16u;
  auto xch = [&](int par, int wave, int dir) __attribute__((always_inline)) -> float* { return lds_x + (((par * 4 + wave) * 2 + dir) * 2 + h) * 16; };
  const int wr = w * 32 + r;
  const int row = (int)blockIdx.x * VALID - HALO + wr;
  const bool inr = row >= 0 && row < p.rows;
  const int row_c = row < 0 ? 0 : (row < p.rows ? row : p.rows - 1);
  const unsigned fl = inr ? p.nbr[row_c] : 0u;
  const float sfl = (fl & 1u) ? UNSCALE : 0.f;
  const float lfl_in = ((fl & 2u) && r != 0) ? UNSCALE : 0.f, rfl_in = ((fl & 4u) && r != 31) ? UNSCALE : 0.f;
  const float lfl_x = ((fl & 2u) && r == 0 && w > 0) ? UNSCALE : 0.f, rfl_x = ((fl & 4u) && r == 31 && w < 3) ? UNSCALE : 0.f;
  const float lfl1 = (fl & 2u) ? 1.f : 0.f, rfl1 = (fl & 4u) ? 1.f : 0.f, sfl1 = (fl & 1u) ? 1.f : 0.f;

  auto issue_piece = [&](const unsigned short* img, int sl, int parity, int i) __attribute__((always_inline)) {
    int pc = w + 4 * i;
    pc = pc < PIECES ? pc : PIECES - 1;
#ifndef DCF_HC_NO_DMA
    glds16(img + ((size_t)sl * PIECES + pc) * 512, lane16, (unsigned)parity * STAGE + (unsigned)pc * 1024u);
#endif
  };
#ifdef DCF_HC_STAMP
  unsigned long long acc_[8] = {0, 0, 0, 0, 0, 0, 0, 0}, last_ = hc_stamp();
#endif
#pragma unroll
  for (int i = 0; i < NPW; ++i) issue_piece(p.W1c, 0, 0, i);

  for (int i = tid; i < C; i += 256) {
    lds_ln[i] = p.ln1_w[i]; lds_ln[C + i] = p.ln1_b[i]; lds_ln[2 * C + i] = p.ln2_w[i]; lds_ln[3 * C + i] = p.ln2_b[i];
  }
#ifdef DCF_HC_VECTOR_OUT
  for (int i = tid; i < NO * 3 * C; i += 256) lds_wo[i] = i < p.NO * 3 * C ? p.Wout[i] : 0.f;
#endif

  constexpr int XA = (256 - 16 * NT - 96) / 8 - 1 > 0 ? (256 - 16 * NT - 96) / 8 - 1 : 0;
  f16x8 xh[KS], xl[KS];
  {
    const float* px = p.X + (int64_t)row_c * p.ldx + 4 * h;
    const bool use = (fl & 1u) != 0;
#pragma unroll
    for (int kk = 0; kk < KS; ++kk) {
#ifndef DCF_HC_NO_X
      f32x4 v0 = *reinterpret_cast<const f32x4*>(px + 16 * kk), v1 = *reinterpret_cast<const f32x4*>(px + 16 * kk + 8);
#else
      f32x4 v0 = f32x4{0.1f, 0.2f, 0.3f, (float)lane}, v1 = f32x4{0.5f, (float)kk, 0.7f, 0.8f};
      (void)px;
#endif
      if (!use) { v0 = f32x4{0.f, 0.f, 0.f, 0.f}; v1 = v0; }
      unsigned hi[4], lo[4];
      split2_f16(v0.x, v0.y, SA, hi[0], lo[0]);
      split2_f16(v0.z, v0.w, SA, hi[1], lo[1]);
      split2_f16(v1.x, v1.y, SA, hi[2], lo[2]);
      split2_f16(v1.z, v1.w, SA, hi[3], lo[3]);
      xh[kk] = __builtin_bit_cast(f16x8, u32x4{hi[0], hi[1], hi[2], hi[3]});
      xl[kk] = __builtin_bit_cast(f16x8, u32x4{lo[0], lo[1], lo[2], lo[3]});
      if (kk < XA) { asm volatile("" : "+a"(xh[kk])); asm volatile("" : "+a"(xl[kk])); }
    }
  }

  STAMP(5);
  f32x16 Y[NT], Z2[2][3];
  bool bad = false;

  auto fixup = [&](auto ot_) __attribute__((always_inline)) {
    constexpr int OT = decltype(ot_)::value;
    const float* pl_ = xch(OT & 1, w > 0 ? w - 1 : 0, 0);
    const float* pr_ = xch(OT & 1, w < 3 ? w + 1 : 3, 1);
#pragma unroll
    for (int g4 = 0; g4 < 4; ++g4) {
      const f32x4 a = *reinterpret_cast<const f32x4*>(pl_ + 4 * g4), b = *reinterpret_cast<const f32x4*>(pr_ + 4 * g4);
#pragma unroll
      for (int i = 0; i < 4; ++i) Y[OT][4 * g4 + i] = __builtin_fmaf(a[i], lfl_x, __builtin_fmaf(b[i], rfl_x, Y[OT][4 * g4 + i]));
    }
    asm volatile("" : "+a"(Y[OT]));
  };

  auto stage = [&](auto ot_, auto hf_, int layer) __attribute__((always_inline)) {
    constexpr int OT = decltype(ot_)::value, HF = decltype(hf_)::value;
    STAMP(2);
    asm volatile("s_waitcnt vmcnt(0)" ::: "memory");
    STAMP(0);
    __syncthreads();
    STAMP(1);
    if constexpr (HF == 1 && OT > 0) fixup(std::integral_constant<int, OT - 1>{});
    unsigned ab = lane16 + HF * STAGE;
    asm volatile("" : "+v"(ab));
    const unsigned char* buf = lds + ab;
    constexpr bool LAST = OT == NT - 1 && HF == 1;
#ifdef DCF_HC_VECTOR_OUT
    const unsigned short* nimg = LAST ? p.W2c : (layer ? p.W2c : p.W1c);
    const bool has_next = !LAST || layer == 0;
#else
    const unsigned short* nimg = LAST ? (layer ? p.Woc : p.W2c) : (layer ? p.W2c : p.W1c);
    const bool has_next = true;
#endif
    const int nsl = LAST ? 0 : 2 * OT + HF + 1;
    f32x16 (&Z)[3] = Z2[OT & 1];
    if constexpr (HF == 0) {
#pragma unroll
      for (int t = 0; t < 3; ++t)
#pragma unroll
        for (int e = 0; e < 16; ++e) Z[t][e] = 0.f;
    }
    f16x8 fa[2][3][2];
    auto frags = [&](int kq, int set) __attribute__((always_inline)) {
#pragma unroll
      for (int tap = 0; tap < 3; ++tap) {
#ifndef DCF_HC_NO_LDS
        fa[set][tap][0] = *reinterpret_cast<const f16x8*>(buf + (2 * (tap * KH + kq)) * 1024);
        fa[set][tap][1] = *reinterpret_cast<const f16x8*>(buf + (2 * (tap * KH + kq) + 1) * 1024);
#else
        fa[set][tap][0] = xh[(kq + tap) % KS]; fa[set][tap][1] = xl[(kq + 2 * tap) % KS];
#endif
      }
    };
    frags(0, 0);
    constexpr int PPG = (NPW + KH - 2) / (KH - 1);
    float t0[4], t1[4], t2[4], p0[4], n2[4];
#pragma unroll
    for (int kq = 0; kq < KH; ++kq) {
      const int set = kq & 1, kk = HF * KH + kq;
      if (kq + 1 < KH) frags(kq + 1, set ^ 1);
      auto piece = [&](int j) __attribute__((always_inline)) {
        const int i = kq * PPG + j;
        if (j < PPG && kq + 1 < KH && i < NPW) {
          if constexpr (LAST) { if (has_next) issue_piece(nimg, nsl, HF ^ 1, i); }
          else issue_piece(nimg, nsl, HF ^ 1, i);
        }
      };
      if (HF == 0 && OT > 0 && kq < 4) {
        f32x16 (&Zp)[3] = Z2[(OT + 1) & 1];
        constexpr int PT = OT > 0 ? OT - 1 : 0;
        const int g4 = kq;
        piece(0);
#pragma unroll
        for (int k = 0; k < 9; ++k) {
          const int tap = k % 3, term = k / 3;
          if (k == 4) piece(1);
          Z[tap] = mma(term == 0 ? fa[set][tap][1] : fa[set][tap][0], term == 1 ? xl[kk] : xh[kk], Z[tap]);
#pragma unroll
          for (int i = 0; i < 4; ++i) {
            if (k == 0) t0[i] = Zp[0][4 * g4 + i];
            if (k == 1) t2[i] = Zp[2][4 * g4 + i];
            if (k == 2) p0[i] = from_prev(t0[i]);
            if (k == 3) n2[i] = from_next(t2[i]);
            if (k == 4) t1[i] = Zp[1][4 * g4 + i] * sfl;
            if (k == 5) t1[i] = __builtin_fmaf(n2[i], rfl_in, t1[i]);
            if (k == 6) t1[i] = __builtin_fmaf(p0[i], lfl_in, t1[i]);
            if (k == 7) Y[PT][4 * g4 + i] = t1[i];
          }
          if (k == 8) {
            if (r == 31) *reinterpret_cast<f32x4*>(xch(PT & 1, w, 0) + 4 * g4) = f32x4{t0[0], t0[1], t0[2], t0[3]};
            if (r == 0) *reinterpret_cast<f32x4*>(xch(PT & 1, w, 1) + 4 * g4) = f32x4{t2[0], t2[1], t2[2], t2[3]};
          }
          const int tn = (k + 1) % 3, pn = (k + 1) / 3 == 0 ? 1 : 0;
#define DCF_HPIN(x) asm volatile("" : "+v"(fa[set][tap][term == 0 ? 1 : 0]), "+v"(fa[set][tn][pn]), "+v"(x[0]), "+v"(x[1]), "+v"(x[2]), "+v"(x[3]))
          if (k == 0) DCF_HPIN(t0);
          if (k == 1) DCF_HPIN(t2);
          if (k == 2) DCF_HPIN(p0);
          if (k == 3) DCF_HPIN(n2);
          if (k >= 4 && k <= 6) DCF_HPIN(t1);
#undef DCF_HPIN
        }
        if (kq == 3) asm volatile("" : "+a"(Y[PT]));
      } else {
      piece(0);
#pragma unroll
      for (int tap = 0; tap < 3; ++tap) Z[tap] = mma(fa[set][tap][1], xh[kk], Z[tap]);
      Z[0] = mma(fa[set][0][0], xl[kk], Z[0]);
      __builtin_amdgcn_sched_barrier(0);
      piece(1);
      Z[1] = mma(fa[set][1][0], xl[kk], Z[1]);
      Z[2] = mma(fa[set][2][0], xl[kk], Z[2]);
#pragma unroll
      for (int tap = 0; tap < 3; ++tap) Z[tap] = mma(fa[set][tap][0], xh[kk], Z[tap]);
      static_assert(PPG <= 2, "two request slots per group");
      }
      __builtin_amdgcn_sched_barrier(0);
    }
    if constexpr (HF == 1 && OT == NT - 1) {
      STAMP(2);
      f32x4 bz0[4], bz2[4];
#pragma unroll
      for (int g4 = 0; g4 < 4; ++g4) {
        float p0[4], n2[4];
#pragma unroll
        for (int i = 0; i < 4; ++i) { bz0[g4][i] = Z[0][4 * g4 + i]; bz2[g4][i] = Z[2][4 * g4 + i]; }
#pragma unroll
        for (int i = 0; i < 4; ++i) { p0[i] = from_prev(bz0[g4][i]); n2[i] = from_next(bz2[g4][i]); }
#pragma unroll
        for (int i = 0; i < 4; ++i) Y[OT][4 * g4 + i] = __builtin_fmaf(p0[i], lfl_in, __builtin_fmaf(n2[i], rfl_in, Z[1][4 * g4 + i] * sfl));
      }
      if (r == 31) {
        float* o = xch(OT & 1, w, 0);
#pragma unroll
        for (int g4 = 0; g4 < 4; ++g4) *reinterpret_cast<f32x4*>(o + 4 * g4) = bz0[g4];
      }
      if (r == 0) {
        float* o = xch(OT & 1, w, 1);
#pragma unroll
        for (int g4 = 0; g4 < 4; ++g4) *reinterpret_cast<f32x4*>(o + 4 * g4) = bz2[g4];
      }
      asm volatile("" : "+a"(Y[OT]));
      STAMP(3);
    }
  };
  auto ln_relu = [&](const float* g, const float* b) __attribute__((always_inline)) {
    float s = 0.f;
#pragma unroll
    for (int ot = 0; ot < NT; ++ot)
#pragma unroll
      for (int e = 0; e < 16; ++e) s += Y[ot][e];
    const float mean = xor32_sum(s) * (1.0f / C);
    bad |= !(__builtin_fabsf(mean) <= 3.4028234664e38f);
    float q = 0.f;
#pragma unroll
    for (int ot = 0; ot < NT; ++ot)
#pragma unroll
      for (int e = 0; e < 16; ++e) { const float d = Y[ot][e] - mean; q = __builtin_fmaf(d, d, q); }
    const float rstd = 1.0f / sqrtf(xor32_sum(q) * (1.0f / C) + 1e-5f);
#pragma unroll
    for (int ot = 0; ot < NT; ++ot)
#pragma unroll
      for (int g4 = 0; g4 < 4; ++g4) {
        const f32x4 gw = *reinterpret_cast<const f32x4*>(g + 32 * ot + 8 * g4 + 4 * h), gb = *reinterpret_cast<const f32x4*>(b + 32 * ot + 8 * g4 + 4 * h);
#pragma unroll
        for (int i = 0; i < 4; ++i) Y[ot][4 * g4 + i] = fmaxf(__builtin_fmaf((Y[ot][4 * g4 + i] - mean) * rstd, gw[i], gb[i]), 0.f);
      }
  };

  for (int layer = 0; layer < 2; ++layer) {
    auto tiles = [&](auto self, auto ot_) __attribute__((always_inline)) -> void {
      constexpr int OT = decltype(ot_)::value;
      if constexpr (OT < NT) {
        stage(ot_, std::integral_constant<int, 0>{}, layer);
        stage(ot_, std::integral_constant<int, 1>{}, layer);
        self(self, std::integral_constant<int, OT + 1>{});
      }
    };
    tiles(tiles, std::integral_constant<int, 0>{});
    STAMP(2);
#ifndef DCF_HC_VECTOR_OUT
    if (layer == 1) asm volatile("s_waitcnt vmcnt(0)" ::: "memory");
#endif
    __syncthreads();
    fixup(std::integral_constant<int, NT - 1>{});
    ln_relu(lds_ln + 2 * C * layer, lds_ln + 2 * C * layer + C);
#ifdef DCF_HC_VECTOR_OUT
    if (layer == 0)
#endif
    {
#pragma unroll
      for (int ot = 0; ot < NT; ++ot)
#pragma unroll
        for (int q = 0; q < 2; ++q) {
          unsigned hi[4], lo[4];
#pragma unroll
          for (int i = 0; i < 4; ++i) split2_f16(Y[ot][8 * q + 2 * i], Y[ot][8 * q + 2 * i + 1], SA, hi[i], lo[i]);
          xh[2 * ot + q] = __builtin_bit_cast(f16x8, u32x4{hi[0], hi[1], hi[2], hi[3]});
          xl[2 * ot + q] = __builtin_bit_cast(f16x8, u32x4{lo[0], lo[1], lo[2], lo[3]});
          if (2 * ot + q < XA) { asm volatile("" : "+a"(xh[2 * ot + q])); asm volatile("" : "+a"(xl[2 * ot + q])); }
        }
    }
  }

  STAMP(4);
#ifdef DCF_HC_VECTOR_OUT
  float pt[3][NO];
#pragma unroll
  for (int t = 0; t < 3; ++t)
#pragma unroll
    for (int o = 0; o < NO; ++o) pt[t][o] = 0.f;
#pragma unroll
  for (int ot = 0; ot < NT; ++ot)
#pragma unroll
    for (int g4 = 0; g4 < 4; ++g4)
#pragma unroll
      for (int o = 0; o < NO; ++o)
#pragma unroll
        for (int t = 0; t < 3; ++t) {
          const f32x4 wv = *reinterpret_cast<const f32x4*>(lds_wo + (o * 3 + t) * C + 32 * ot + 8 * g4 + 4 * h);
          pt[t][o] += (Y[ot][4 * g4] * wv.x + Y[ot][4 * g4 + 1] * wv.y) + (Y[ot][4 * g4 + 2] * wv.z + Y[ot][4 * g4 + 3] * wv.w);
        }
  float d0[NO], d1[NO], d2[NO];
#pragma unroll
  for (int o = 0; o < NO; ++o) { d0[o] = xor32_sum(pt[0][o]); d1[o] = xor32_sum(pt[1][o]); d2[o] = xor32_sum(pt[2][o]); }
#else
  float d0[NO], d1[NO], d2[NO];
  {
    f32x16 (&T3)[3] = Z2[0];
#pragma unroll
    for (int t = 0; t < 3; ++t)
#pragma unroll
      for (int e = 0; e < 16; ++e) T3[t][e] = 0.f;
    const unsigned char* buf = lds + lane16;
#pragma unroll
    for (int kk = 0; kk < KS; ++kk) {
      const f16x8 ah = *reinterpret_cast<const f16x8*>(buf + (2 * kk) * 1024), al = *reinterpret_cast<const f16x8*>(buf + (2 * kk + 1) * 1024);
      T3[0] = mma(al, xh[kk], T3[0]);
      T3[1] = mma(ah, xl[kk], T3[1]);
      T3[2] = mma(ah, xh[kk], T3[2]);
    }
#pragma unroll
    for (int o = 0; o < NO; ++o) {
      d0[o] = ((T3[0][o] + T3[1][o]) + T3[2][o]) * UNSCALE;
      d1[o] = ((T3[0][2 + o] + T3[1][2 + o]) + T3[2][2 + o]) * UNSCALE;
      d2[o] = ((T3[0][4 + o] + T3[1][4 + o]) + T3[2][4 + o]) * UNSCALE;
    }
    bad |= h == 0 && !(__builtin_fabsf((d0[0] + d0[1]) + (d1[0] + d1[1]) + (d2[0] + d2[1])) <= 3.4028234664e38f);
  }
#endif
  __syncthreads();
  if (h == 0) {
#pragma unroll
    for (int o = 0; o < NO; ++o) {
      if (r == 31) lds_x[(w * 2 + 0) * 2 + o] = d0[o];
      if (r == 0) lds_x[(w * 2 + 1) * 2 + o] = d2[o];
    }
  }
  __syncthreads();
  float yo[NO];
#pragma unroll
  for (int o = 0; o < NO; ++o) {
    const float xl_ = lds_x[((w > 0 ? w - 1 : 0) * 2 + 0) * 2 + o], xr_ = lds_x[((w < 3 ? w + 1 : 3) * 2 + 1) * 2 + o];
    const float sp = from_prev(d0[o]), sn = from_next(d2[o]);
    const float pv = r == 0 ? (w > 0 ? xl_ : 0.f) : sp;
    const float nx = r == 31 ? (w < 3 ? xr_ : 0.f) : sn;
    yo[o] = __builtin_fmaf(pv, lfl1, __builtin_fmaf(nx, rfl1, d1[o] * sfl1)) + (o < p.NO ? p.bout[o] : 0.f);
  }
  if (h == 0 && wr >= HALO && wr < HALO + VALID && inr) {
    const LevelTable* lt = p.lt;
    const int l = find_level_hc(lt, row);
    int64_t dst = row;
    if (p.query_major) {
      const int rel = row - lt->start[l];
      const int b = rel / lt->T[l], t = rel - b * lt->T[l];
      dst = (int64_t)b * lt->S + lt->off[l] + t;
    }
#pragma unroll
    for (int o = 0; o < NO; ++o) {
      float y = yo[o];
      if (p.mode == 1) y = fmaxf(y * lt->scale[l], 0.f);
      if (o < p.NO) p.out[dst * p.NO + o] = y;
    }
  }
  if (bad && p.status) atomicOr(p.status, 1u);
#ifdef DCF_HC_STAMP
  STAMP(6);
#ifndef DCF_HC_STAMP_WG
#define DCF_HC_STAMP_WG 1
#endif
  if (blockIdx.x == DCF_HC_STAMP_WG && blockIdx.y == 0 && tid == 0)
    for (int i = 0; i < 8; ++i) dcf_hc_stamps[i] = acc_[i];
#endif
}

#ifdef DCF_HC_STAMP
}
extern "C" int dcf_debug_hc_stamps(unsigned long long* out) {
  return hipMemcpyFromSymbol(out, HIP_SYMBOL(dcf::dcf_hc_stamps), 8 * sizeof(unsigned long long)) == hipSuccess ? 0 : -1;
}
namespace dcf {
#endif

bool head_chain_supports(int C, int NO) { return (C == 256 || C == 288) && (NO == 1 || NO == 2); }

size_t head_chain_out_image_halfs(int C) { return (size_t)(3 * (C / 32) * 2) * 512; }

int launch_split_chain_out(const float* Wout, int NO, unsigned short* img, int C, hipStream_t stream, unsigned* overflow) {
  DCF_CHECK((C == 256 || C == 288) && (NO == 1 || NO == 2), "launch_split_chain_out: C = %d, NO = %d", C, NO);
  DCF_HIP(hipMemsetAsync(img, 0, head_chain_out_image_halfs(C) * sizeof(unsigned short), stream));
  const int n = 6 * (C / 2);
  if (C == 256) hipLaunchKernelGGL(k_split_chain_out<256>, dim3((n + 255) / 256), dim3(256), 0, stream, Wout, NO, img, overflow);
  else hipLaunchKernelGGL(k_split_chain_out<288>, dim3((n + 255) / 256), dim3(256), 0, stream, Wout, NO, img, overflow);
  DCF_HIP(hipGetLastError());
  return 0;
}

size_t head_chain_image_halfs(int C) { return (size_t)(C / 32) * 2 * (3 * (C / 32) * 2) * 512; }

int launch_split_chain3(const float* Wp, unsigned short* img, int C, hipStream_t stream, unsigned* overflow) {
  DCF_CHECK(C == 256 || C == 288, "launch_split_chain3: C = %d (256 or 288)", C);
  const int n = C * 3 * (C / 2);
  if (C == 256) hipLaunchKernelGGL(k_split_chain3<256>, dim3((n + 255) / 256), dim3(256), 0, stream, Wp, img, overflow);
  else hipLaunchKernelGGL(k_split_chain3<288>, dim3((n + 255) / 256), dim3(256), 0, stream, Wp, img, overflow);
  DCF_HIP(hipGetLastError());
  return 0;
}

template <int C>
static int launch_hc(const HeadChainArgs* a, int count, hipStream_t stream) {
#ifdef DCF_HC_VECTOR_OUT
  constexpr int bytes = 2 * Geo<C>::STAGE + (4 * C + 2 * 3 * C + 2 * 4 * 2 * 2 * 16) * (int)sizeof(float);
#else
  constexpr int bytes = 2 * Geo<C>::STAGE + (4 * C + 2 * 4 * 2 * 2 * 16) * (int)sizeof(float);
  static_assert(2 * Geo<C>::KS <= Geo<C>::PIECES, "the image of the output convolution fits a stage");
#endif
  if (raise_lds_limit<&k_head_chain<C>>(bytes)) return -1;
  HeadChainBatch b{};
  for (int i = 0; i < count; ++i) b.a[i] = a[i];
  const unsigned grid = (unsigned)((a[0].rows + VALID - 1) / VALID);
  hipLaunchKernelGGL((k_head_chain<C>), dim3(grid, (unsigned)count), dim3(256), bytes, stream, b);
  DCF_HIP(hipGetLastError());
  return 0;
}

int launch_head_chain(const HeadChainArgs* a, int count, int C, hipStream_t stream) {
  DCF_CHECK(count == 1 || count == 2, "launch_head_chain: one or two heads per launch");
  for (int i = 0; i < count; ++i) {
    DCF_CHECK(head_chain_supports(C, a[i].NO), "launch_head_chain: C = %d, NO = %d (C 256 / 288, NO 1 / 2)", C, a[i].NO);
    DCF_CHECK(a[i].rows > 0 && a[i].rows == a[0].rows && a[i].X && a[i].nbr && a[i].W1c && a[i].W2c && a[i].ln1_w && a[i].ln1_b && a[i].ln2_w &&
                  a[i].ln2_b && a[i].Wout && a[i].bout && a[i].lt && a[i].out, "launch_head_chain: null argument or unequal row counts");
    DCF_CHECK((reinterpret_cast<uintptr_t>(a[i].X) & 15) == 0 && a[i].ldx % 4 == 0 && (reinterpret_cast<uintptr_t>(a[i].W1c) & 15) == 0 &&
                  (reinterpret_cast<uintptr_t>(a[i].W2c) & 15) == 0, "launch_head_chain: X / weight images must be 16-byte aligned");
    DCF_CHECK(a[i].Woc && (reinterpret_cast<uintptr_t>(a[i].Woc) & 15) == 0, "launch_head_chain: no image of the output convolution, or not 16-byte aligned");
  }
  return C == 256 ? launch_hc<256>(a, count, stream) : launch_hc<288>(a, count, stream);
}

}
```

### cvpr2025-decafnet_amd/csrc/ops_api.hip

```cpp
#include <algorithm>

#include "engine.h"

namespace dcf {
static int split_gemm_once(GemmArgs g, GemmAMode mode, int nterms, hipStream_t st) {
  StreamScratch sc(st);
  unsigned short* planes = nullptr;
  if (sc.take(&planes, (size_t)3 * g.N * g.K)) return -1;
  int rc = launch_split_planes(g.W, planes, g.N, g.K, g.K, st, nterms);
  g.Ws = planes;
  if (rc == 0) rc = launch_gemm_split(&g, 1, mode, nterms, st);
  return sc.end(rc);
}
static int conv3_once(const float* X, const uint8_t* mask, const float* W_ock, float* Y, int B, int T, int Cin, int N, int nterms,
                      hipStream_t st) {
  const int rows = B * T;
  StreamScratch sc(st);
  float* wp = nullptr;
  uint8_t* nbr = nullptr;
  unsigned short* planes = nullptr;
  if (sc.take(&wp, (size_t)N * Cin * 3) || sc.take(&nbr, (size_t)rows)) return -1;
  if (nterms && sc.take(&planes, (size_t)3 * N * Cin * 3)) return -1;
  launch_permute3(W_ock, wp, N, Cin, 3, 0, 2, 1, st);
  int rc = launch_rowflags(mask, nbr, T, rows, st);
  if (rc == 0 && nterms) rc = launch_split_planes(wp, planes, N, 3 * Cin, 3 * Cin, st, nterms);
  if (rc == 0) {
    GemmArgs g = gemm(X, Cin, wp, nullptr, Y, N, rows, N, 3 * Cin);
    g.cin = Cin; g.nbr = nbr; g.Ws = planes;
    rc = nterms ? launch_gemm_split(&g, 1, A_ROWS_TAP3, nterms, st) : launch_gemm(&g, 1, A_ROWS_TAP3, st);
  }
  return sc.end(rc);
}
}

extern "C" {

int dcf_collect_segments(const float* logits, const float* offsets, const uint8_t* masks, int32_t nq, int64_t T,
                         int32_t n_levels, float pre_nms_thresh, int32_t pre_nms_topk, float seg_len_thresh,
                         float* segs_out, float* scores_out, int32_t* counts_out, void* stream) {
  return dcf_collect_segments_ext(logits, offsets, masks, nullptr, nq, T, n_levels, pre_nms_thresh, pre_nms_topk, seg_len_thresh,
                                  segs_out, scores_out, counts_out, stream);
}

int dcf_collect_segments_ext(const float* logits, const float* offsets, const uint8_t* masks, const float* ext_scores,
                             int32_t nq, int64_t T, int32_t n_levels, float pre_nms_thresh, int32_t pre_nms_topk,
                             float seg_len_thresh, float* segs_out, float* scores_out, int32_t* counts_out, void* stream) {
  DCF_CHECK(logits && offsets && masks && segs_out && scores_out && counts_out, "dcf_collect_segments: null argument");
  DCF_CHECK(n_levels >= 1 && n_levels <= 16, "dcf_collect_segments: n_levels out of range");
  dcf::CollectArgs a{};
  a.logits = logits; a.offsets = offsets; a.masks = masks;
  a.ext = ext_scores; a.T = (int)T;
  int acc = 0;
  for (int l = 0; l < n_levels; ++l) { a.off[l] = acc; acc += (int)(T >> l); }
  a.off[n_levels] = acc;
  a.S = acc; a.n_levels = n_levels;
  a.pre_nms_thresh = pre_nms_thresh; a.seg_len_thresh = seg_len_thresh; a.pre_nms_topk = pre_nms_topk;
  a.segs = segs_out; a.scores = scores_out; a.counts = counts_out;
  dcf::StreamScratch sc((hipStream_t)stream);
  uint32_t* keys = nullptr;
  if (dcf::collect_needs_scratch(acc) && sc.take(&keys, (size_t)nq * acc)) return -1;
  a.keys = keys;
  return sc.end(dcf::launch_collect(a, nq, (hipStream_t)stream));
}

int dcf_nms_1d(const float* segs, const float* scores, const int32_t* counts, int32_t nq, int32_t n_max,
               int32_t stride, float iou_thresh, int64_t* keep_out, int32_t* keep_counts_out, void* stream) {
  DCF_CHECK(keep_out && keep_counts_out && (n_max == 0 || (segs && scores)), "dcf_nms_1d: null argument");
  dcf::NmsArgs a{segs, scores, counts, n_max, stride, iou_thresh, (long long*)keep_out, keep_counts_out};
  return dcf::launch_nms(a, nq, (hipStream_t)stream);
}

int dcf_softnms_1d(const float* segs, const float* scores, const int32_t* counts, int32_t nq, int32_t n_max,
                   int32_t stride, float iou_thresh, float sigma, float min_score, int32_t method,
                   int32_t max_iters, float* dets_out, int64_t* inds_out, int32_t* out_counts, void* stream) {
  DCF_CHECK(dets_out && inds_out && out_counts && (n_max == 0 || (segs && scores)), "dcf_softnms_1d: null argument");
  dcf::SoftNmsArgs a{segs, scores, counts, n_max, stride, iou_thresh, sigma, min_score, method, max_iters, dets_out,
                     (long long*)inds_out, out_counts};
  return dcf::launch_softnms(a, nq, (hipStream_t)stream);
}

int dcf_segment_voting(const float* nms_segs, int32_t nms_ld, const int32_t* n1_counts, int32_t n1_max,
                       int32_t n1_stride, const float* all_segs, const float* all_scores,
                       const int32_t* n2_counts, int32_t n2_max, int32_t n2_stride, float iou_thresh,
                       int32_t nq, float* out, void* stream) {
// ... 288 lines not shown
  int rc = resolve_encoder(m, prefix, c.E, st, w);
  ScratchArena sa;
  if (rc == 0) {
    Buffers b{};
    const size_t need = carve_at(nullptr, c, T, B, B, T, 1, 1, b);
    if (hipMalloc(&sa.base, need) != hipSuccess) { set_error("dcf_op_encoder: out of memory"); rc = -1; }
    if (rc == 0) {
      carve_at(sa.base, c, T, B, B, T, 1, 1, b);
      if (stride == 2) rc = launch_mask_down(mask, mask_out, B * T / 2, st);
      else if (hipMemcpyAsync(mask_out, mask, (size_t)B * T, hipMemcpyDeviceToDevice, st) != hipSuccess) rc = -1;
      if (rc == 0) rc = run_encoder(m, w, b, X, c.E, mask, mask_out, B, T, stride, Y, c.E, st);
    }
  }
  return scratch_end(m, st, rc);
}

int dcf_op_enc_pre(dcf_model* m, const char* prefix, const float* X, const uint8_t* mask, int32_t B, int32_t T, int32_t stride,
                   float* Qc, float* Kc, float* Vc, float* Skip, void* stream) {
  using namespace dcf;
  hipStream_t st = (hipStream_t)stream;
  DCF_CHECK(prefix && X && mask && Qc && Kc && Vc && B >= 1 && T >= 1 && (stride == 1 || (stride == 2 && Skip)) && T % stride == 0, "dcf_op_enc_pre: bad arguments");
  if (scratch_begin(m, "dcf_op_enc_pre", st)) return -1;
  EncW w{};
  int rc = resolve_encoder(m, prefix, m->cfg.E, st, w);
  if (rc == 0) {
    EncPreArgs ep = enc_pre_args(w, X, m->cfg.E, mask, B, T, m->cfg.E);
    ep.Qc = Qc; ep.Kc = Kc; ep.Vc = Vc; ep.Skip = stride == 2 ? Skip : nullptr;
    rc = launch_enc_pre(ep, stride, st);
  }
  return scratch_end(m, st, rc);
}

int dcf_op_decoder(dcf_model* m, const char* prefix, float* X, const uint8_t* mask, int32_t B, int32_t T,
                   const float* const* text, const uint8_t* const* text_mask, const int32_t* text_len, void* stream) {
  using namespace dcf;
  hipStream_t st = (hipStream_t)stream;
  DCF_CHECK(prefix && X && mask && text && text_len && B >= 1 && B <= DCF_MAX_BATCH && T >= 1, "dcf_op_decoder: bad arguments");
  if (scratch_begin(m, "dcf_op_decoder", st)) return -1;
  const dcf_config& c = m->cfg;
  DecW w{};
  int rc = resolve_decoder(m, prefix, c.E, c.TE, st, w);
  ScratchArena sa;
  if (rc == 0) {
    m->dec.assign(1, w);
    m->fus_out_w = m->fus_out_b = nullptr;
    int Lk = 1;
    TextMeta tm{};
    for (int i = 0; i < B; ++i) {
      tm.text[i] = text[i]; tm.text_mask[i] = text_mask ? text_mask[i] : nullptr; tm.len[i] = text_len[i];
      Lk = std::max(Lk, (int)text_len[i]);
    }
    Buffers b{};
    const size_t need = carve_at(nullptr, c, T, B, B, T, Lk, 1, b);
    if (hipMalloc(&sa.base, need) != hipSuccess) { set_error("dcf_op_decoder: out of memory"); rc = -1; }
    if (rc == 0) carve_at(sa.base, c, T, B, B, T, Lk, 1, b);
    if (rc == 0) rc = run_fusion(m, b, X, c.E, B, T, nullptr, mask, nullptr, &tm, Lk, X, c.E, st);
  }
  return scratch_end(m, st, rc);
}

int dcf_op_tcn(dcf_model* m, const char* prefix, const float* x, const uint8_t* mask, int32_t B, int32_t T, int32_t n_in,
               int32_t n_layers, float* Y, void* stream) {
  using namespace dcf;
  hipStream_t st = (hipStream_t)stream;
  DCF_CHECK(prefix && x && mask && Y && B >= 1 && T >= 1 && n_in >= 1 && n_in <= DCF_MAX_LEVELS && n_layers >= 0, "dcf_op_tcn: bad arguments");
  if (scratch_begin(m, "dcf_op_tcn", st)) return -1;
  int rc = resolve_tcn(m, prefix, n_in, n_layers, st);
  float* buf = nullptr;
  if (rc == 0 && hipMalloc(&buf, (size_t)2 * B * T * TCN_HID * sizeof(float)) != hipSuccess) { set_error("dcf_op_tcn: out of memory"); rc = -1; }
  if (rc == 0) {
    LevelTable lt{};
    lt.n_levels = n_in; lt.B = B; lt.T[0] = T; lt.S = T;
    RefineArgs ra = refine_args(m);
    ra.stacked = x; ra.mask_all = mask;
    ra.bufA = buf; ra.bufB = buf + (size_t)B * T * TCN_HID; ra.F = Y; ra.ldf = TCN_HID; ra.E = 0;
    ra.B = B; ra.T0 = T; ra.n_levels = n_in; ra.n_layers = n_layers;
    rc = launch_refine(ra, lt, st);
  }
  rc = scratch_end(m, st, rc);
  if (buf) (void)hipFree(buf);
  return rc;
}

}
```

Baseline: 21.59 million clips/s.

## Fuse embedding FC and two tap-3 convolutions into one windowed chain kernel

Folds the embedding linear layer (and optional input LayerNorm affine) into the first 3-tap embedding convolution at load time. The folded conv, LN+ReLU, second conv, LN+ReLU and position encoding then run in a single windowed kernel reusing the head-chain machinery with a 2-row halo. This removes several full-sequence GEMM and LayerNorm launches and their intermediate activation round trips through memory. The costs are recomputed halo rows, a shared kernel body that is more complex, and a fallback to the old path if the folded weights overflow the scaled fp16 range. It also adds a debug 'gemm_uniform' option that is off by default.

```diff
diff --git a/cvpr2025-decafnet_amd/_lib.py b/cvpr2025-decafnet_amd/_lib.py
--- a/cvpr2025-decafnet_amd/_lib.py
+++ b/cvpr2025-decafnet_amd/_lib.py
@@ -204,6 +204,13 @@
 }
 
 
+EMBD_SIGNATURES = {
+    'dcf_embd_ext_version': (i32, []),
+    'dcf_op_embd_chain': (i32, [vp, c_f32p, i64, c_u8p, i32, i32, i32, c_f32p, c_f32p, i64, vp]),
+    'dcf_op_embd_launches': (i32, [vp, c_f32p, i64, c_u8p, i32, i32, i32, c_f32p, c_f32p, i64, vp]),
+}
+
+
 def lib():
     global _LIB
     if _LIB is None:
@@ -214,7 +221,7 @@
         h = ctypes.CDLL(SO_PATH, mode=ctypes.RTLD_GLOBAL)
         for name, (res, args) in list(SIGNATURES.items()) + list(TRAIN_SIGNATURES.items()) + list(DIST_SIGNATURES.items()) + \
                 list(ATTN_SIGNATURES.items()) + list(FRONT_SIGNATURES.items()) + list(GUARD_SIGNATURES.items()) + list(CLOCK_SIGNATURES.items()) + \
-                list(HALF_SIGNATURES.items()) + list(FRONT_HALF_SIGNATURES.items()):
+                list(HALF_SIGNATURES.items()) + list(FRONT_HALF_SIGNATURES.items()) + list(EMBD_SIGNATURES.items()):
             fn = getattr(h, name)
             fn.restype = res
             fn.argtypes = args
diff --git a/cvpr2025-decafnet_amd/csrc/embd_chain.h b/cvpr2025-decafnet_amd/csrc/embd_chain.h
--- /dev/null
+++ b/cvpr2025-decafnet_amd/csrc/embd_chain.h
@@ -0,0 +1,26 @@
+#pragma once
+#include <hip/hip_runtime.h>
+#include <stdint.h>
+
+namespace dcf {
+
+struct EmbdChainArgs {
+  const float* X;
+  int64_t ldx;
+  const uint8_t* nbr;
+  const unsigned short* W1c;
+  const unsigned short* W2c;
+  const float* cb;
+  const float* ln1_w; const float* ln1_b; const float* ln2_w; const float* ln2_b;
+  const float* pe;
+  float* Y;
+  int64_t ldy;
+  int rows, T;
+  int ln_in;
+  unsigned* status;
+};
+
+bool embd_chain_supports(int C);
+int launch_embd_chain(const EmbdChainArgs& a, hipStream_t stream);
+
+}
diff --git a/cvpr2025-decafnet_amd/csrc/engine.h b/cvpr2025-decafnet_amd/csrc/engine.h
--- a/cvpr2025-decafnet_amd/csrc/engine.h
+++ b/cvpr2025-decafnet_amd/csrc/engine.h
@@ -9,6 +9,7 @@
 #include "common.h"
 #include "dec_chain.h"
 #include "dropout.h"
+#include "embd_chain.h"
 #include "enc_chain.h"
 #include "ffn_chain.h"
 #include "gemm.h"
@@ -96,6 +97,9 @@
   const float *embd_fc_w = nullptr, *embd_fc_b = nullptr;
   const float *embd_fc_wf = nullptr, *embd_fc_s = nullptr, *embd_fc_c = nullptr;
   std::vector<const float*> embd_conv, embd_ln_w, embd_ln_b;
+  const unsigned short* embd_chain_w1[2] = {nullptr, nullptr};
+  const float* embd_chain_cb[2] = {nullptr, nullptr};
+  const unsigned short* embd_chain_w2 = nullptr;
   std::vector<dcf::EncW> stem, branch;
   std::vector<const float*> pool_w;
   dcf::HeadW cls1, cls2, reg;
@@ -258,6 +262,9 @@
 int run_fusion_drop(dcf_model* m, Buffers& b, float* X, int64_t ldx, int B, int T, const uint8_t* mask, const TextMeta* dm, int Lk,
                     float* out, int64_t ld_out, hipStream_t st);
 RefineArgs refine_args(dcf_model* m);
+bool can_chain_embd(dcf_model* m, int rows0);
+int run_embd_chain(dcf_model* m, const float* X, int64_t ldx, const uint8_t* nbr, int rows, int T, bool ln_in, const float* pe, float* Y,
+                   int64_t ldy, hipStream_t st);
 
 int forward(dcf_model* m, const VideoSet& vs, int T0, int nq, const ForwardCall& fc, hipStream_t st);
 void launch_masks_out(const uint8_t* mask_all, uint8_t* out, const LevelTable* lt, const unsigned* status, float* logits, int rows,
diff --git a/cvpr2025-decafnet_amd/csrc/engine.hip b/cvpr2025-decafnet_amd/csrc/engine.hip
--- a/cvpr2025-decafnet_amd/csrc/engine.hip
+++ b/cvpr2025-decafnet_amd/csrc/engine.hip
@@ -287,6 +287,11 @@
     }
 
     {
+      const bool chain_embd = can_chain_embd(m, rows0);
+      if (chain_embd) {
+        TRY(run_embd_chain(m, fused_as_stats ? b.X : b.R[0], E, b.nbr_all, rows0, T0, fused_as_stats, c.use_abs_pe ? m->pe : nullptr, b.R[3], E, st));
+        std::swap(b.X, b.R[3]);
+      } else
       if (c.model_kind != 1 && fused_as_stats) {
         GemmArgs ge = gemm(b.X, E, m->embd_fc_wf, m->embd_fc_c, b.R[3], E, rows0, E, E);
         ge.flags = G_AMASK; ge.rowmask = mask0;
@@ -321,7 +326,7 @@
         DCF_CHECK(Tc == Tp, "vid_net.arch[0]=%d embedding convolutions cannot divide the sequence by vid_net.stride=%d (video_net.py:53)", c.n_embd_convs, sv);
       }
       int epend = -1, epend_w = 0;
-      for (int i = 0; i < c.n_embd_convs && sv == 1; ++i) {
+      for (int i = 0; i < c.n_embd_convs && sv == 1 && !chain_embd; ++i) {
         GemmArgs g = gemm(b.X, E, m->embd_conv[i], nullptr, b.R[0], E, rows0, E, 3 * E);
         g.cin = E; g.nbr = b.nbr_all;
         const bool with_pe = c.use_abs_pe && i == c.n_embd_convs - 1;
diff --git a/cvpr2025-decafnet_amd/csrc/engine_blocks.hip b/cvpr2025-decafnet_amd/csrc/engine_blocks.hip
--- a/cvpr2025-decafnet_amd/csrc/engine_blocks.hip
+++ b/cvpr2025-decafnet_amd/csrc/engine_blocks.hip
@@ -569,6 +569,25 @@
   return launch_ln(ln, st);
 }
 
+bool can_chain_embd(dcf_model* m, int rows0) {
+  static const Setting off(nullptr, "DCF_NO_EMBD_CHAIN", 0, Setting::PRESENT);
+  static const Setting min_rows("embd_chain_min_rows", "DCF_EMBD_CHAIN_MIN_ROWS", 16384);
+  const dcf_config& c = m->cfg;
+  return !off.get() && debug_option("embd_chain", 1) != 0 && m->gemm_terms == GEMM_F16X3 && c.E == 256 && c.model_kind != 1 &&
+         vid_stride_of(c) == 1 && c.n_embd_convs == 2 && !m->drop && !m->keep_debug && m->embd_chain_w1[0] && m->embd_chain_w1[1] &&
+         m->embd_chain_w2 && rows0 >= min_rows.get();
+}
+int run_embd_chain(dcf_model* m, const float* X, int64_t ldx, const uint8_t* nbr, int rows, int T, bool ln_in, const float* pe, float* Y,
+                   int64_t ldy, hipStream_t st) {
+  const int E = m->cfg.E, v = ln_in ? 0 : 1;
+  EmbdChainArgs a{};
+  a.X = X; a.ldx = ldx; a.nbr = nbr; a.W1c = m->embd_chain_w1[v]; a.W2c = m->embd_chain_w2; a.cb = m->embd_chain_cb[v];
+  a.ln1_w = m->embd_ln_w[0]; a.ln1_b = m->embd_ln_b[0]; a.ln2_w = m->embd_ln_w[1]; a.ln2_b = m->embd_ln_b[1];
+  a.pe = pe; a.Y = Y; a.ldy = ldy; a.rows = rows; a.T = T; a.ln_in = ln_in ? 1 : 0; a.status = m->status;
+  ProfScope prof("gemm_f16x3<embd_chain>", st, 2.0 * rows * 256.0 * 768.0 * 2.0, (double)rows * E * 4.0 * 2.0);
+  return launch_embd_chain(a, st);
+}
+
 RefineArgs refine_args(dcf_model* m) {
   static const Setting stack("tcn_stack", "DCF_TCN_STACK", -1);
   RefineArgs ra{};
diff --git a/cvpr2025-decafnet_amd/csrc/engine_model.hip b/cvpr2025-decafnet_amd/csrc/engine_model.hip
--- a/cvpr2025-decafnet_amd/csrc/engine_model.hip
+++ b/cvpr2025-decafnet_amd/csrc/engine_model.hip
@@ -98,6 +98,28 @@
 void launch_fold_ln(const float* W, const float* bias, const float* g, const float* beta, float* Wf, float* s, float* c, int N, int K,
                     hipStream_t st) {
   hipLaunchKernelGGL(k_fold_ln, dim3(N), dim3(64), 0, st, W, bias, g, beta, Wf, s, c, K);
+}
+
+__global__ void k_fold_embd_d(const float* __restrict__ Wfc, const float* __restrict__ bfc, const float* __restrict__ beta, double* __restrict__ d, int E) {
+  const int j = blockIdx.x * blockDim.x + threadIdx.x;
+  if (j >= E) return;
+  double a = bfc[j];
+  if (beta)
+    for (int k = 0; k < E; ++k) a += (double)Wfc[(int64_t)j * E + k] * (double)beta[k];
+  d[j] = a;
+}
+__global__ void k_fold_embd(const float* __restrict__ Wc, const float* __restrict__ Wfc, const float* __restrict__ g, const double* __restrict__ d,
+                            float* __restrict__ Wf, float* __restrict__ cb, int E) {
+  const int n = blockIdx.x / 3, tap = blockIdx.x - 3 * n, k = threadIdx.x;
+  const float* wc = Wc + ((int64_t)n * 3 + tap) * E;
+  double a = 0.;
+  for (int j = 0; j < E; ++j) a += (double)wc[j] * (double)Wfc[(int64_t)j * E + k];
+  Wf[((int64_t)n * 3 + tap) * E + k] = (float)(g ? a * (double)g[k] : a);
+  if (k == 0) {
+    double c = 0.;
+    for (int j = 0; j < E; ++j) c += (double)wc[j] * d[j];
+    cb[(int64_t)tap * E + n] = (float)c;
+  }
 }
 
 void drop_graph(dcf_model* m, bool keep_last_key) {
@@ -472,6 +494,31 @@
     GET("vid_net.embd_norms." + s + ".weight", SH(E), lw); GET("vid_net.embd_norms." + s + ".bias", SH(E), lb);
     m->embd_ln_w.push_back(lw); m->embd_ln_b.push_back(lb);
   }
+  m->embd_chain_w1[0] = m->embd_chain_w1[1] = m->embd_chain_w2 = nullptr;
+  m->embd_chain_cb[0] = m->embd_chain_cb[1] = nullptr;
+  unsigned* embd_overflow = nullptr;
+  if (m->gemm_terms == GEMM_F16X3 && c.model_kind != 1 && vid_stride_of(c) == 1 && c.n_embd_convs == 2 && embd_chain_supports(E)) {
+    const size_t img = head_chain_image_halfs(E) * sizeof(unsigned short), wf = (size_t)E * 3 * E * sizeof(float);
+    char* buf = nullptr;
+    DCF_HIP(hipMalloc(&buf, 3 * img + 2 * 3 * E * sizeof(float) + 256 + wf + E * sizeof(double)));
+    m->owned.push_back(reinterpret_cast<float*>(buf));
+    unsigned short* imgs[3] = {reinterpret_cast<unsigned short*>(buf), reinterpret_cast<unsigned short*>(buf + img), reinterpret_cast<unsigned short*>(buf + 2 * img)};
+    float* cb = reinterpret_cast<float*>(buf + 3 * img);
+    embd_overflow = reinterpret_cast<unsigned*>(cb + 2 * 3 * E);
+    float* Wf = reinterpret_cast<float*>(buf + 3 * img + 2 * 3 * E * sizeof(float) + 256);
+    double* d = reinterpret_cast<double*>(reinterpret_cast<char*>(Wf) + wf);
+    DCF_HIP(hipMemsetAsync(embd_overflow, 0, sizeof(unsigned), st));
+    for (int v = 0; v < 2; ++v) {
+      const float *g = v == 0 ? m->fus_out_w : nullptr, *beta = v == 0 ? m->fus_out_b : nullptr;
+      hipLaunchKernelGGL(k_fold_embd_d, dim3((E + 255) / 256), dim3(256), 0, st, m->embd_fc_w, m->embd_fc_b, beta, d, E);
+      hipLaunchKernelGGL(k_fold_embd, dim3(3 * E), dim3(E), 0, st, m->embd_conv[0], m->embd_fc_w, g, (const double*)d, Wf, cb + v * 3 * E, E);
+      DCF_HIP(hipGetLastError());
+      if (launch_split_chain3(Wf, imgs[v], E, st, embd_overflow)) return -1;
+      m->embd_chain_w1[v] = imgs[v]; m->embd_chain_cb[v] = cb + v * 3 * E;
+    }
+    if (launch_split_chain3(m->embd_conv[1], imgs[2], E, st, nullptr)) return -1;
+    m->embd_chain_w2 = imgs[2];
+  }
   for (int i = 0; i < c.n_stem; ++i) {
     EncW w{};
     if (resolve_encoder(m, "vid_net.stem." + std::to_string(i), E, st, w)) return -1;
@@ -501,6 +548,11 @@
   }
   if (c.model_kind == 0 && resolve_tcn(m, "refine", L, L, st)) return -1;
   DCF_HIP(hipStreamSynchronize(st));
+  if (embd_overflow) {
+    unsigned over = 0u;
+    DCF_HIP(hipMemcpy(&over, embd_overflow, sizeof(over), hipMemcpyDeviceToHost));
+    if (over) m->embd_chain_w1[0] = m->embd_chain_w1[1] = m->embd_chain_w2 = nullptr;
+  }
   for (auto& pl : m->plans) if (pl.d_lt) (void)hipFree(pl.d_lt);
   m->plans.clear();
   free_hybrid(m);
@@ -633,7 +685,7 @@
 
 int dcf_debug_set_option(const char* name, int32_t value) {
   DCF_CHECK(name && *name, "dcf_debug_set_option: empty name");
-  static const char* known[] = {"dec_chain_min_rows", "enc_chain_min_rows", "enc_attn_min_rows", "fuse_scores", "tcn_frag", "gate_skip", "tcn_stack", "half_native"};
+  static const char* known[] = {"dec_chain_min_rows", "enc_chain_min_rows", "enc_attn_min_rows", "fuse_scores", "tcn_frag", "gate_skip", "tcn_stack", "half_native", "embd_chain", "embd_chain_min_rows", "gemm_uniform"};
   bool ok = false;
   for (const char* k : known) ok = ok || strcmp(k, name) == 0;
   DCF_CHECK(ok, "dcf_debug_set_option: unknown option '%s'", name);
diff --git a/cvpr2025-decafnet_amd/csrc/gemm_bf16s.hip b/cvpr2025-decafnet_amd/csrc/gemm_bf16s.hip
--- a/cvpr2025-decafnet_amd/csrc/gemm_bf16s.hip
+++ b/cvpr2025-decafnet_amd/csrc/gemm_bf16s.hip
@@ -745,8 +745,11 @@
   return 0;
 }
 
+int debug_option(const char* name, int dflt);
+static bool gemm_uniform() { return debug_option("gemm_uniform", 0) != 0; }
+
 bool gemm_can_fuse_adaln(int M, int N, int K) {
-  if (N % 256 != 0 || K % SBK != 0) return false;
+  if (N % 256 != 0 || K % SBK != 0 || gemm_uniform()) return false;
   const long tiles64 = (long)((M + 63) / 64) * (N / 64);
   if (K >= 4 * SBK && tiles64 <= 512) return false;
   return M >= 65536 || (long)((M + 63) / 64) * (N / 256) >= 448;
@@ -754,6 +757,7 @@
 
 bool gemm_can_carry_stats(int M, int N, int K, int count, int nterms) {
   if (nterms == 0 || N % 64 != 0 || K % SBK != 0 || M <= 0) return false;
+  if (gemm_uniform()) return true;
   const long tiles64 = (long)((M + 63) / 64) * (N / 64) * count;
   constexpr long kslice_max = 512;
   if (K >= 4 * SBK && tiles64 <= ((K >= 16 * SBK && nterms != T_F16) ? kslice_max : kslice_max / 2)) return false;
@@ -761,13 +765,14 @@
 }
 
 bool gemm_can_norm_a(int M, int N, int K, int nterms, int* stats_w) {
-  if (nterms == 0 || K % SBK != 0 || M <= 0) return false;
+  if (nterms == 0 || K % SBK != 0 || M <= 0 || gemm_uniform()) return false;
   if (N % 256 == 0 && M >= 65536) { if (stats_w) *stats_w = 64; return true; }
   (void)nterms;
   return false;
 }
 
 bool gemm_can_fuse_ln(int M, int N, int K, GemmAMode mode) {
+  if (gemm_uniform()) return false;
   constexpr long min_tiles = 448;
   return mode != A_CHANMAJOR && mode != A_CHANMAJOR_H && N == 256 && K % SBK == 0 && (M + 63) / 64 >= min_tiles;
 }
@@ -824,13 +829,15 @@
       if (bm == 128 && bn == 256) return launch_cfg_s<1, 4, 4, 2>(b, count, mode, nterms, stream);
     }
   }
+  const bool uniform = gemm_uniform();
+  if (uniform && !p.ln_w && N % 128 == 0) return launch_cfg_s<1, 4, 2, 1>(b, count, mode, nterms, stream);
   if (p.ln_w) {
     DCF_CHECK(count == 1 && p.Y && p.ln_b && gemm_can_fuse_ln(p.M, N, p.K, mode), "launch_gemm_split: LayerNorm cannot be fused for %dx%dx%d", p.M, N, p.K);
     if (p.ln_pe) DCF_CHECK(p.ln_mask && p.ln_T >= 64, "launch_gemm_split: fused position encoding needs a mask and T >= 64");
     return launch_cfg_s<1, 4, 2, 2>(b, count, mode, nterms, stream);
   }
   constexpr long kslice_max = 512;
-  if (mode == A_ROWS && N % 64 == 0 && p.K >= 4 * SBK && wgs(64, 64) <= ((p.K >= 16 * SBK && nterms != T_F16) ? kslice_max : kslice_max / 2))
+  if (!uniform && mode == A_ROWS && N % 64 == 0 && p.K >= 4 * SBK && wgs(64, 64) <= ((p.K >= 16 * SBK && nterms != T_F16) ? kslice_max : kslice_max / 2))
     return launch_kslice(b, count, nterms, stream);
   if (mode == A_CHANMAJOR || mode == A_CHANMAJOR_H) {
     DCF_CHECK(N % 128 == 0, "launch_gemm_split: channel-major A needs N %% 128 == 0");
diff --git a/cvpr2025-decafnet_amd/csrc/head_chain.hip b/cvpr2025-decafnet_amd/csrc/head_chain.hip
--- a/cvpr2025-decafnet_amd/csrc/head_chain.hip
+++ b/cvpr2025-decafnet_amd/csrc/head_chain.hip
@@ -3,6 +3,7 @@
 #include <type_traits>
 
 #include "common.h"
+#include "embd_chain.h"
 
 namespace dcf {
 
@@ -14,7 +15,11 @@
 typedef unsigned u32x4 __attribute__((ext_vector_type(4)));
 
 constexpr float SA = 16.f, SW = 256.f, UNSCALE = 1.f / 4096.f;
-constexpr int HALO = 3, WGROWS = 128, VALID = WGROWS - 2 * HALO;
+constexpr int WGROWS = 128;
+template <bool EMBD>
+struct Win {
+  static constexpr int HALO = EMBD ? 2 : 3, VALID = WGROWS - 2 * HALO;
+};
 
 template <int C>
 struct Geo {
@@ -114,32 +119,38 @@
 }
 
 struct HeadChainBatch { HeadChainArgs a[2]; };
-template <int C>
-__global__ __launch_bounds__(256, 1) void k_head_chain(HeadChainBatch batch) {
+template <int C, class Args>
+__device__ __forceinline__ void chain_body(const Args& p) {
+  constexpr bool EMBD = std::is_same<Args, EmbdChainArgs>::value;
   constexpr int NO = 2;
-  const HeadChainArgs& p = batch.a[blockIdx.y];
+  constexpr int HALO = Win<EMBD>::HALO, VALID = Win<EMBD>::VALID;
   using G = Geo<C>;
   constexpr int KS = G::KS, KH = G::KH, NT = G::NT, STAGE = G::STAGE, PIECES = G::PIECES, NPW = G::NPW;
   extern __shared__ __attribute__((aligned(16))) unsigned char lds[];
   float* lds_ln = reinterpret_cast<float*>(lds + 2 * STAGE);
 #ifdef DCF_HC_VECTOR_OUT
+  static_assert(!EMBD, "DCF_HC_VECTOR_OUT is an A/B build of the heads");
   float* lds_wo = lds_ln + 4 * C;
   float* lds_x = lds_wo + NO * 3 * C;
-#else
-  float* lds_x = lds_ln + 4 * C;
+  float* lds_cb = nullptr;
+#else
+  float* lds_cb = lds_ln + 4 * C;
+  float* lds_x = lds_ln + (EMBD ? 7 : 4) * C;
 #endif
   const int tid = threadIdx.x, lane = tid & 63, r = lane & 31, h = lane >> 5;
   const int w = __builtin_amdgcn_readfirstlane(tid >> 6);
   const unsigned lane16 = (unsigned)lane * 16u;
-  auto xch = [&](int par, int wave, int dir) __attribute__((always_inline)) -> float* { return lds_x + (((par * 4 + wave) * 2 + dir) * 2 + h) * 16; };
+  constexpr int ND = EMBD ? 3 : 2;
+  auto xch = [&](int par, int wave, int dir) __attribute__((always_inline)) -> float* { return lds_x + (((par * 4 + wave) * ND + dir) * 2 + h) * 16; };
   const int wr = w * 32 + r;
   const int row = (int)blockIdx.x * VALID - HALO + wr;
   const bool inr = row >= 0 && row < p.rows;
   const int row_c = row < 0 ? 0 : (row < p.rows ? row : p.rows - 1);
   const unsigned fl = inr ? p.nbr[row_c] : 0u;
   const float sfl = (fl & 1u) ? UNSCALE : 0.f;
-  const float lfl_in = ((fl & 2u) && r != 0) ? UNSCALE : 0.f, rfl_in = ((fl & 4u) && r != 31) ? UNSCALE : 0.f;
-  const float lfl_x = ((fl & 2u) && r == 0 && w > 0) ? UNSCALE : 0.f, rfl_x = ((fl & 4u) && r == 31 && w < 3) ? UNSCALE : 0.f;
+  const bool l_late = EMBD && r == 31;
+  const float lfl_in = ((fl & 2u) && r != 0 && !l_late) ? UNSCALE : 0.f, rfl_in = ((fl & 4u) && r != 31) ? UNSCALE : 0.f;
+  const float lfl_x = ((fl & 2u) && ((r == 0 && w > 0) || l_late)) ? UNSCALE : 0.f, rfl_x = ((fl & 4u) && r == 31 && w < 3) ? UNSCALE : 0.f;
   const float lfl1 = (fl & 2u) ? 1.f : 0.f, rfl1 = (fl & 4u) ? 1.f : 0.f, sfl1 = (fl & 1u) ? 1.f : 0.f;
 
   auto issue_piece = [&](const unsigned short* img, int sl, int parity, int i) __attribute__((always_inline)) {
@@ -157,6 +168,7 @@
 
   for (int i = tid; i < C; i += 256) {
     lds_ln[i] = p.ln1_w[i]; lds_ln[C + i] = p.ln1_b[i]; lds_ln[2 * C + i] = p.ln2_w[i]; lds_ln[3 * C + i] = p.ln2_b[i];
+    if constexpr (EMBD) { lds_cb[i] = p.cb[i]; lds_cb[C + i] = p.cb[C + i]; lds_cb[2 * C + i] = p.cb[2 * C + i]; }
   }
 #ifdef DCF_HC_VECTOR_OUT
   for (int i = tid; i < NO * 3 * C; i += 256) lds_wo[i] = i < p.NO * 3 * C ? p.Wout[i] : 0.f;
@@ -164,7 +176,43 @@
 
   constexpr int XA = (256 - 16 * NT - 96) / 8 - 1 > 0 ? (256 - 16 * NT - 96) / 8 - 1 : 0;
   f16x8 xh[KS], xl[KS];
-  {
+  if constexpr (EMBD) {
+    const float* px = p.X + (int64_t)row_c * p.ldx + 4 * h;
+    const bool use = (fl & 1u) != 0;
+    f32x4 v[KS][2];
+#pragma unroll
+    for (int kk = 0; kk < KS; ++kk) {
+      v[kk][0] = *reinterpret_cast<const f32x4*>(px + 16 * kk); v[kk][1] = *reinterpret_cast<const f32x4*>(px + 16 * kk + 8);
+      if (!use) { v[kk][0] = f32x4{0.f, 0.f, 0.f, 0.f}; v[kk][1] = v[kk][0]; }
+    }
+    float s = 0.f;
+#pragma unroll
+    for (int kk = 0; kk < KS; ++kk)
+#pragma unroll
+      for (int i = 0; i < 4; ++i) s += v[kk][0][i] + v[kk][1][i];
+    const float mean = xor32_sum(s) * (1.0f / C);
+    float q = 0.f;
+#pragma unroll
+    for (int kk = 0; kk < KS; ++kk)
+#pragma unroll
+      for (int i = 0; i < 4; ++i) {
+        const float d0 = v[kk][0][i] - mean, d1 = v[kk][1][i] - mean;
+        q = __builtin_fmaf(d0, d0, q); q = __builtin_fmaf(d1, d1, q);
+      }
+    const float rstd = 1.0f / sqrtf(xor32_sum(q) * (1.0f / C) + 1e-5f);
+    const float mu = p.ln_in ? mean : 0.f, rs = p.ln_in ? rstd : 1.f;
+#pragma unroll
+    for (int kk = 0; kk < KS; ++kk) {
+      unsigned hi[4], lo[4];
+      split2_f16((v[kk][0].x - mu) * rs, (v[kk][0].y - mu) * rs, SA, hi[0], lo[0]);
+      split2_f16((v[kk][0].z - mu) * rs, (v[kk][0].w - mu) * rs, SA, hi[1], lo[1]);
+      split2_f16((v[kk][1].x - mu) * rs, (v[kk][1].y - mu) * rs, SA, hi[2], lo[2]);
+      split2_f16((v[kk][1].z - mu) * rs, (v[kk][1].w - mu) * rs, SA, hi[3], lo[3]);
+      xh[kk] = __builtin_bit_cast(f16x8, u32x4{hi[0], hi[1], hi[2], hi[3]});
+      xl[kk] = __builtin_bit_cast(f16x8, u32x4{lo[0], lo[1], lo[2], lo[3]});
+      if (kk < XA) { asm volatile("" : "+a"(xh[kk])); asm volatile("" : "+a"(xl[kk])); }
+    }
+  } else {
     const float* px = p.X + (int64_t)row_c * p.ldx + 4 * h;
     const bool use = (fl & 1u) != 0;
 #pragma unroll
@@ -193,7 +241,7 @@
 
   auto fixup = [&](auto ot_) __attribute__((always_inline)) {
     constexpr int OT = decltype(ot_)::value;
-    const float* pl_ = xch(OT & 1, w > 0 ? w - 1 : 0, 0);
+    const float* pl_ = l_late ? xch(OT & 1, w, 2) : xch(OT & 1, w > 0 ? w - 1 : 0, 0);
     const float* pr_ = xch(OT & 1, w < 3 ? w + 1 : 3, 1);
 #pragma unroll
     for (int g4 = 0; g4 < 4; ++g4) {
@@ -220,8 +268,14 @@
     const unsigned short* nimg = LAST ? p.W2c : (layer ? p.W2c : p.W1c);
     const bool has_next = !LAST || layer == 0;
 #else
-    const unsigned short* nimg = LAST ? (layer ? p.Woc : p.W2c) : (layer ? p.W2c : p.W1c);
-    const bool has_next = true;
+    const unsigned short* nimg;
+    bool has_next = true;
+    if constexpr (EMBD) {
+      nimg = layer ? p.W2c : (LAST ? p.W2c : p.W1c);
+      has_next = !LAST || layer == 0;
+    } else {
+      nimg = LAST ? (layer ? p.Woc : p.W2c) : (layer ? p.W2c : p.W1c);
+    }
 #endif
     const int nsl = LAST ? 0 : 2 * OT + HF + 1;
     f32x16 (&Z)[3] = Z2[OT & 1];
@@ -280,6 +334,7 @@
           }
           if (k == 8) {
             if (r == 31) *reinterpret_cast<f32x4*>(xch(PT & 1, w, 0) + 4 * g4) = f32x4{t0[0], t0[1], t0[2], t0[3]};
+            if constexpr (EMBD) { if (r == 31) *reinterpret_cast<f32x4*>(xch(PT & 1, w, 2) + 4 * g4) = f32x4{p0[0], p0[1], p0[2], p0[3]}; }
             if (r == 0) *reinterpret_cast<f32x4*>(xch(PT & 1, w, 1) + 4 * g4) = f32x4{t2[0], t2[1], t2[2], t2[3]};
           }
           const int tn = (k + 1) % 3, pn = (k + 1) / 3 == 0 ? 1 : 0;
@@ -319,6 +374,7 @@
         for (int i = 0; i < 4; ++i) { p0[i] = from_prev(bz0[g4][i]); n2[i] = from_next(bz2[g4][i]); }
 #pragma unroll
         for (int i = 0; i < 4; ++i) Y[OT][4 * g4 + i] = __builtin_fmaf(p0[i], lfl_in, __builtin_fmaf(n2[i], rfl_in, Z[1][4 * g4 + i] * sfl));
+        if constexpr (EMBD) { if (r == 31) *reinterpret_cast<f32x4*>(xch(OT & 1, w, 2) + 4 * g4) = f32x4{p0[0], p0[1], p0[2], p0[3]}; }
       }
       if (r == 31) {
         float* o = xch(OT & 1, w, 0);
@@ -374,11 +430,27 @@
 #endif
     __syncthreads();
     fixup(std::integral_constant<int, NT - 1>{});
+    if constexpr (EMBD) {
+      if (layer == 0) {
+#pragma unroll
+        for (int ot = 0; ot < NT; ++ot)
+#pragma unroll
+          for (int g4 = 0; g4 < 4; ++g4) {
+            const float* pc = lds_cb + 32 * ot + 8 * g4 + 4 * h;
+            const f32x4 c0 = *reinterpret_cast<const f32x4*>(pc), c1 = *reinterpret_cast<const f32x4*>(pc + C), c2 = *reinterpret_cast<const f32x4*>(pc + 2 * C);
+#pragma unroll
+            for (int i = 0; i < 4; ++i)
+              Y[ot][4 * g4 + i] += __builtin_fmaf(c0[i], lfl1, __builtin_fmaf(c2[i], rfl1, c1[i] * sfl1));
+          }
+      }
+    }
     ln_relu(lds_ln + 2 * C * layer, lds_ln + 2 * C * layer + C);
+    bool split = true;
 #ifdef DCF_HC_VECTOR_OUT
-    if (layer == 0)
-#endif
-    {
+    split = layer == 0;
+#endif
+    if constexpr (EMBD) split = layer == 0;
+    if (split) {
 #pragma unroll
       for (int ot = 0; ot < NT; ++ot)
 #pragma unroll
@@ -394,6 +466,24 @@
   }
 
   STAMP(4);
+  if constexpr (EMBD) {
+    const bool with_pe = p.pe != nullptr;
+    const int t = with_pe ? row_c % p.T : 0;
+    const float* ppe = (with_pe ? p.pe + (int64_t)t * C : p.ln2_w) + 4 * h;
+    float* py = p.Y + (int64_t)row_c * p.ldy + 4 * h;
+    const bool keep = wr >= HALO && wr < HALO + VALID && inr;
+#pragma unroll
+    for (int ot = 0; ot < NT; ++ot)
+#pragma unroll
+      for (int g4 = 0; g4 < 4; ++g4) {
+        f32x4 e = *reinterpret_cast<const f32x4*>(ppe + 32 * ot + 8 * g4);
+        if (!with_pe) e = f32x4{0.f, 0.f, 0.f, 0.f};
+        f32x4 o;
+#pragma unroll
+        for (int i = 0; i < 4; ++i) o[i] = __builtin_fmaf(e[i], sfl1, Y[ot][4 * g4 + i]);
+        if (keep) *reinterpret_cast<f32x4*>(py + 32 * ot + 8 * g4) = o;
+      }
+  } else {
 #ifdef DCF_HC_VECTOR_OUT
   float pt[3][NO];
 #pragma unroll
@@ -473,6 +563,7 @@
       if (o < p.NO) p.out[dst * p.NO + o] = y;
     }
   }
+  }
   if (bad && p.status) atomicOr(p.status, 1u);
 #ifdef DCF_HC_STAMP
   STAMP(6);
@@ -483,6 +574,16 @@
     for (int i = 0; i < 8; ++i) dcf_hc_stamps[i] = acc_[i];
 #endif
 }
+
+template <int C>
+__global__ __launch_bounds__(256, 1) void k_head_chain(HeadChainBatch batch) {
+  chain_body<C>(batch.a[blockIdx.y]);
+}
+#ifndef DCF_HC_VECTOR_OUT
+__global__ __launch_bounds__(256, 1) void k_embd_chain(EmbdChainArgs a) {
+  chain_body<256>(a);
+}
+#endif
 
 #ifdef DCF_HC_STAMP
 }
@@ -528,7 +629,7 @@
   if (raise_lds_limit<&k_head_chain<C>>(bytes)) return -1;
   HeadChainBatch b{};
   for (int i = 0; i < count; ++i) b.a[i] = a[i];
-  const unsigned grid = (unsigned)((a[0].rows + VALID - 1) / VALID);
+  const unsigned grid = (unsigned)((a[0].rows + Win<false>::VALID - 1) / Win<false>::VALID);
   hipLaunchKernelGGL((k_head_chain<C>), dim3(grid, (unsigned)count), dim3(256), bytes, stream, b);
   DCF_HIP(hipGetLastError());
   return 0;
@@ -547,4 +648,26 @@
   return C == 256 ? launch_hc<256>(a, count, stream) : launch_hc<288>(a, count, stream);
 }
 
-}
+bool embd_chain_supports(int C) { return C == 256; }
+
+int launch_embd_chain(const EmbdChainArgs& a, hipStream_t stream) {
+#ifdef DCF_HC_VECTOR_OUT
+  DCF_CHECK(false, "launch_embd_chain: not in a DCF_HC_VECTOR_OUT build");
+#else
+  constexpr int C = 256;
+  DCF_CHECK(a.rows > 0 && a.T > 0 && a.X && a.nbr && a.W1c && a.W2c && a.cb && a.ln1_w && a.ln1_b && a.ln2_w && a.ln2_b && a.Y, "launch_embd_chain: null argument");
+  DCF_CHECK(a.X != a.Y, "launch_embd_chain: not in place (neighbouring windows read each other's halo rows)");
+  DCF_CHECK((reinterpret_cast<uintptr_t>(a.X) & 15) == 0 && a.ldx % 4 == 0 && a.ldx >= C && (reinterpret_cast<uintptr_t>(a.Y) & 15) == 0 && a.ldy % 4 == 0 &&
+                a.ldy >= C && (reinterpret_cast<uintptr_t>(a.W1c) & 15) == 0 && (reinterpret_cast<uintptr_t>(a.W2c) & 15) == 0 &&
+                (reinterpret_cast<uintptr_t>(a.pe) & 15) == 0 && (reinterpret_cast<uintptr_t>(a.ln2_w) & 15) == 0,
+            "launch_embd_chain: X / Y / pe / ln2_w / weight images must be 16-byte aligned, the row pitches multiples of 4 and >= %d", C);
+  constexpr int bytes = 2 * Geo<C>::STAGE + (7 * C + 2 * 4 * 3 * 2 * 16) * (int)sizeof(float);
+  if (raise_lds_limit<&k_embd_chain>(bytes)) return -1;
+  const unsigned grid = (unsigned)((a.rows + Win<true>::VALID - 1) / Win<true>::VALID);
+  hipLaunchKernelGGL(k_embd_chain, dim3(grid), dim3(256), bytes, stream, a);
+  DCF_HIP(hipGetLastError());
+  return 0;
+#endif
+}
+
+}
diff --git a/cvpr2025-decafnet_amd/csrc/ops_api.hip b/cvpr2025-decafnet_amd/csrc/ops_api.hip
--- a/cvpr2025-decafnet_amd/csrc/ops_api.hip
+++ b/cvpr2025-decafnet_amd/csrc/ops_api.hip
@@ -1,5 +1,6 @@
 #include <algorithm>
 
+#include "../../include/decafnet_hip_embd.h"
 #include "engine.h"
 
 namespace dcf {
@@ -454,4 +455,67 @@
   return rc;
 }
 
-}
+int dcf_embd_ext_version(void) { return DCF_EMBD_EXT_VERSION; }
+
+static int embd_op_check(const dcf_model* m, const char* what, const float* X, int64_t ldx, const uint8_t* mask, int B, int T, const float* Y, int64_t ldy) {
+  DCF_CHECK(m && X && mask && Y && B >= 1 && T >= 1 && (int64_t)B * T < (1ll << 31), "%s: null argument or bad B / T", what);
+  DCF_CHECK(m->finalized, "%s: the model is not finalized", what);
+  const dcf_config& c = m->cfg;
+  DCF_CHECK(c.model_kind != 1 && dcf::vid_stride_of(c) == 1 && c.n_embd_convs == 2 && c.E == 256 && m->gemm_terms == dcf::GEMM_F16X3,
+            "%s: needs an early-fusion model with E = 256, vid_net.stride 1 and two embedding convolutions in the f16x3 mode", what);
+  DCF_CHECK(X != Y && ldx >= c.E && ldy >= c.E && ldx % 4 == 0 && ldy % 4 == 0, "%s: X and Y must differ, pitches multiples of 4 and >= E", what);
+  return 0;
+}
+
+int dcf_op_embd_chain(dcf_model* m, const float* X, int64_t ldx, const uint8_t* mask, int32_t B, int32_t T, int32_t ln_in,
+                      const float* pe, float* Y, int64_t ldy, void* stream) {
+  hipStream_t st = (hipStream_t)stream;
+  if (embd_op_check(m, "dcf_op_embd_chain", X, ldx, mask, B, T, Y, ldy)) return -1;
+  DCF_CHECK(m->embd_chain_w1[0] && m->embd_chain_w1[1] && m->embd_chain_w2,
+            "dcf_op_embd_chain: the model has no images of the folded embedding stage (a folded weight left the scaled fp16 range)");
+  const int rows = B * T;
+  dcf::StreamScratch sc(st);
+  uint8_t* nbr = nullptr;
+  if (sc.take(&nbr, (size_t)rows)) return -1;
+  int rc = dcf::launch_rowflags(mask, nbr, T, rows, st);
+  if (rc == 0) rc = dcf::run_embd_chain(m, X, ldx, nbr, rows, T, ln_in != 0, pe, Y, ldy, st);
+  return sc.end(rc);
+}
+
+int dcf_op_embd_launches(dcf_model* m, const float* X, int64_t ldx, const uint8_t* mask, int32_t B, int32_t T, int32_t ln_in,
+                         const float* pe, float* Y, int64_t ldy, void* stream) {
+  using namespace dcf;
+  hipStream_t st = (hipStream_t)stream;
+  if (embd_op_check(m, "dcf_op_embd_launches", X, ldx, mask, B, T, Y, ldy)) return -1;
+  const int rows = B * T, E = m->cfg.E;
+  StreamScratch sc(st);
+  uint8_t* nbr = nullptr;
+  float *t0 = nullptr, *t1 = nullptr;
+  if (sc.take(&nbr, (size_t)rows) || sc.take(&t0, (size_t)rows * E) || sc.take(&t1, (size_t)rows * E)) return -1;
+  int rc = launch_rowflags(mask, nbr, T, rows, st);
+  const float* xin = X;
+  int64_t ldin = ldx;
+  if (rc == 0 && ln_in) {
+    LnArgs ln{}; ln.X = X; ln.ldx = ldx; ln.Y = t0; ln.ldy = E; ln.w = m->fus_out_w; ln.b = m->fus_out_b; ln.rows = rows; ln.C = E;
+    rc = launch_ln(ln, st);
+    xin = t0; ldin = E;
+  }
+  if (rc == 0) {
+    GemmArgs ge = gemm(xin, ldin, m->embd_fc_w, m->embd_fc_b, t1, E, rows, E, E);
+    ge.flags = G_AMASK; ge.rowmask = mask;
+    rc = run_gemm(m, &ge, 1, A_ROWS, st);
+  }
+  for (int i = 0; i < 2 && rc == 0; ++i) {
+    GemmArgs g = gemm(t1, E, m->embd_conv[i], nullptr, t0, E, rows, E, 3 * E);
+    g.cin = E; g.nbr = nbr;
+    rc = run_gemm(m, &g, 1, A_ROWS_TAP3, st);
+    if (rc) break;
+    LnArgs ln{}; ln.X = t0; ln.ldx = E; ln.Y = i == 1 ? Y : t1; ln.ldy = i == 1 ? ldy : E; ln.w = m->embd_ln_w[i]; ln.b = m->embd_ln_b[i];
+    ln.rows = rows; ln.C = E; ln.relu = 1;
+    if (i == 1 && pe) { ln.pe = pe; ln.mask = mask; ln.T = T; }
+    rc = launch_ln(ln, st);
+  }
+  return sc.end(rc);
+}
+
+}
diff --git a/include/decafnet_hip_embd.h b/include/decafnet_hip_embd.h
--- /dev/null
+++ b/include/decafnet_hip_embd.h
@@ -0,0 +1,25 @@
+#ifndef DECAFNET_HIP_EMBD_H
+#define DECAFNET_HIP_EMBD_H
+
+#include <stdint.h>
+
+#include "decafnet_hip.h"
+
+#ifdef __cplusplus
+extern "C" {
+#endif
+
+#define DCF_EMBD_EXT_VERSION 1
+
+int dcf_embd_ext_version(void);
+
+int dcf_op_embd_chain(dcf_model* model, const float* X, int64_t ldx, const uint8_t* mask, int32_t B, int32_t T, int32_t ln_in,
+                      const float* pe, float* Y, int64_t ldy, void* stream);
+
+int dcf_op_embd_launches(dcf_model* model, const float* X, int64_t ldx, const uint8_t* mask, int32_t B, int32_t T, int32_t ln_in,
+                         const float* pe, float* Y, int64_t ldy, void* stream);
+
+#ifdef __cplusplus
+}
+#endif
+#endif
```

After: 21.93 million clips/s, median of 6. 1.02x the previous value.
